# HeyWeCome/WhisprRec

Measured on AMD Instinct MI355X. Metric: BPR training triplets/sec, higher is better.
Workload: dtype f32; 1 GPU; BPRMF emb_size=64, synthetic 1000000 users x 1000000 items (uniform ids), batch 65536, SGD l2=0, plan build in timed region; batch=65536, emb_size=64, optimizer=SGD, plan_chunk_batches=64, tables=single GPU, step_stream=whisprrec_amd.hip_ops.PipelinedSgd, plan=group plan (no per-batch sort: flags + lists of the shared rows, wr_group.hip), chained_step_launch=True, plan_build=on a side stream, beside the steps of the chunk before

## Files before the change

### include/whisprrec_hip.h

```cpp
#ifndef WHISPRREC_HIP_H
#define WHISPRREC_HIP_H

#include <stdint.h>

#ifdef __cplusplus
extern "C" {
#endif

#define WR_ABI_VERSION 1

#define WR_OK 0
#define WR_E_NULL (-1)
#define WR_E_SHAPE (-2)
#define WR_E_WORKSPACE (-3)
#define WR_E_ALIGN (-4)
#define WR_E_RANGE (-5)

int32_t wr_abi_version(void);
const char *wr_last_error(void);
int32_t wr_device_info(int32_t *n_cu, int32_t *wave_size, char *arch, int32_t arch_len);

int64_t wr_bpr_fwd_workspace_bytes(int64_t B);
int32_t wr_bpr_fwd(const float *user_tab, int64_t n_users, const float *item_tab, int64_t n_items, int32_t D,
                   const int64_t *u, const int64_t *p, const int64_t *n, int64_t B, float *pos_score, float *neg_score,
// ... 5 lines not shown
                                int32_t *tn, int32_t *torig, int32_t *oc_item, int32_t *oc_src, int32_t *err_flag,
                                void *workspace, int64_t workspace_bytes, void *stream);
int32_t wr_bprmf_plan_build_i32(const int32_t *u, const int32_t *p, const int32_t *n, int64_t n_triplets,
                                int64_t batch_size, int64_t n_users, int64_t n_items, int32_t *tu, int32_t *tp,
                                int32_t *tn, int32_t *torig, int32_t *oc_item, int32_t *oc_src, int32_t *err_flag,
                                void *workspace, int64_t workspace_bytes, void *stream);

int64_t wr_bprmf_plan_small_max_batch(void);
int32_t wr_bprmf_plan_build_small_i64(const int64_t *u, const int64_t *p, const int64_t *n, int64_t n_triplets,
                                      int64_t batch_size, int64_t n_users, int64_t n_items, int32_t *tu, int32_t *tp,
                                      int32_t *tn, int32_t *torig, int32_t *oc_item, int32_t *oc_src, int32_t *err_flag,
                                      void *stream);
int32_t wr_bprmf_plan_build_small_i32(const int32_t *u, const int32_t *p, const int32_t *n, int64_t n_triplets,
                                      int64_t batch_size, int64_t n_users, int64_t n_items, int32_t *tu, int32_t *tp,
                                      int32_t *tn, int32_t *torig, int32_t *oc_item, int32_t *oc_src, int32_t *err_flag,
                                      void *stream);

int64_t wr_bprmf_plan_fast_workspace_bytes(int64_t n_triplets, int64_t batch_size, int64_t n_users, int64_t n_items);
int32_t wr_bprmf_plan_build_fast_i64(const int64_t *u, const int64_t *p, const int64_t *n, int64_t n_triplets,
                                     int64_t batch_size, int64_t n_users, int64_t n_items, int32_t *tu, int32_t *tp,
                                     int32_t *tn, int32_t *torig, int32_t *oc_item, int32_t *oc_src, int32_t *flags,
                                     void *workspace, int64_t workspace_bytes, void *stream);
int32_t wr_bprmf_plan_build_fast_i32(const int32_t *u, const int32_t *p, const int32_t *n, int64_t n_triplets,
                                     int64_t batch_size, int64_t n_users, int64_t n_items, int32_t *tu, int32_t *tp,
                                     int32_t *tn, int32_t *torig, int32_t *oc_item, int32_t *oc_src, int32_t *flags,
                                     void *workspace, int64_t workspace_bytes, void *stream);

int32_t wr_bprmf_plan_fast_marks_supported(int64_t n_triplets, int64_t batch_size, int64_t n_users, int64_t n_items);
int32_t wr_bprmf_plan_build_fast_marks_i64(const int64_t *u, const int64_t *p, const int64_t *n, int64_t n_triplets,
                                           int64_t batch_size, int64_t n_users, int64_t n_items, int32_t *tu, int32_t *tp,
                                           int32_t *tn, int32_t *torig, int32_t *oc_item, int32_t *oc_src, int32_t *flags,
                                           void *workspace, int64_t workspace_bytes, int32_t *bitmap, void *stream);
int32_t wr_bprmf_plan_build_fast_marks_i32(const int32_t *u, const int32_t *p, const int32_t *n, int64_t n_triplets,
                                           int64_t batch_size, int64_t n_users, int64_t n_items, int32_t *tu, int32_t *tp,
                                           int32_t *tn, int32_t *torig, int32_t *oc_item, int32_t *oc_src, int32_t *flags,
                                           void *workspace, int64_t workspace_bytes, int32_t *bitmap, void *stream);

typedef struct wr_bucket_side {
    int32_t n_buckets;
    const int32_t *row_bucket;
    const int32_t *bucket_start;
    const int32_t *bucket_rows;
    const int32_t *bucket_sub;
} wr_bucket_side;

int64_t wr_bprmf_plan_fast_mapped_workspace_bytes(int64_t n_triplets, int64_t batch_size, int64_t n_users, int64_t n_items,
                                                  int32_t n_buckets_users, int32_t n_buckets_items);
int32_t wr_bprmf_plan_build_fast_mapped_i64(const int64_t *u, const int64_t *p, const int64_t *n, int64_t n_triplets,
                                            int64_t batch_size, int64_t n_users, int64_t n_items,
                                            const wr_bucket_side *map_users, const wr_bucket_side *map_items, int32_t *tu,
                                            int32_t *tp, int32_t *tn, int32_t *torig, int32_t *oc_item, int32_t *oc_src,
                                            int32_t *flags, void *workspace, int64_t workspace_bytes, void *stream);
int32_t wr_bprmf_plan_build_fast_mapped_i32(const int32_t *u, const int32_t *p, const int32_t *n, int64_t n_triplets,
                                            int64_t batch_size, int64_t n_users, int64_t n_items,
                                            const wr_bucket_side *map_users, const wr_bucket_side *map_items, int32_t *tu,
                                            int32_t *tp, int32_t *tn, int32_t *torig, int32_t *oc_item, int32_t *oc_src,
                                            int32_t *flags, void *workspace, int64_t workspace_bytes, void *stream);

int32_t wr_sample_negatives_i64(const int64_t *users, int64_t n, int64_t n_users, int64_t n_items, const int64_t *clicked_ptr,
                                const int32_t *clicked_idx, uint64_t seed, uint64_t epoch, int64_t *neg_items,
                                int32_t *err_flag, void *stream);
int32_t wr_sample_negatives_i32(const int32_t *users, int64_t n, int64_t n_users, int64_t n_items, const int64_t *clicked_ptr,
                                const int32_t *clicked_idx, uint64_t seed, uint64_t epoch, int32_t *neg_items,
                                int32_t *err_flag, void *stream);

int32_t wr_epoch_prepare_range_i64(const int64_t *users, const int64_t *items, int64_t n, int64_t n_users, int64_t n_items,
                                   const int64_t *clicked_ptr, const int32_t *clicked_idx, uint64_t seed, uint64_t epoch,
                                   int64_t first, int64_t count, int64_t *out_users, int64_t *out_pos, int64_t *out_neg,
                                   int64_t *order_out, int32_t *err_flag, void *stream);
int32_t wr_epoch_prepare_range_i32(const int32_t *users, const int32_t *items, int64_t n, int64_t n_users, int64_t n_items,
                                   const int64_t *clicked_ptr, const int32_t *clicked_idx, uint64_t seed, uint64_t epoch,
                                   int64_t first, int64_t count, int32_t *out_users, int32_t *out_pos, int32_t *out_neg,
                                   int64_t *order_out, int32_t *err_flag, void *stream);

int64_t wr_pairset_capacity(int64_t n_pairs);
int32_t wr_pairset_build(const int64_t *clicked_ptr, const int32_t *clicked_idx, int64_t n_users, uint64_t *table,
                         int64_t capacity, int32_t *err_flag, void *stream);
int32_t wr_sample_negatives_set_i64(const int64_t *users, int64_t n, int64_t n_users, int64_t n_items, const uint64_t *pair_table,
                                    int64_t pair_capacity, uint64_t seed, uint64_t epoch, int64_t *neg_items,
                                    int32_t *err_flag, void *stream);
int32_t wr_sample_negatives_set_i32(const int32_t *users, int64_t n, int64_t n_users, int64_t n_items, const uint64_t *pair_table,
                                    int64_t pair_capacity, uint64_t seed, uint64_t epoch, int32_t *neg_items,
                                    int32_t *err_flag, void *stream);
int32_t wr_epoch_prepare_range_set_i64(const int64_t *users, const int64_t *items, int64_t n, int64_t n_users, int64_t n_items,
                                       const uint64_t *pair_table, int64_t pair_capacity, uint64_t seed, uint64_t epoch,
                                       int64_t first, int64_t count, int64_t *out_users, int64_t *out_pos, int64_t *out_neg,
                                       int64_t *order_out, int32_t *err_flag, void *stream);
int32_t wr_epoch_prepare_range_set_i32(const int32_t *users, const int32_t *items, int64_t n, int64_t n_users, int64_t n_items,
                                       const uint64_t *pair_table, int64_t pair_capacity, uint64_t seed, uint64_t epoch,
                                       int64_t first, int64_t count, int32_t *out_users, int32_t *out_pos, int32_t *out_neg,
                                       int64_t *order_out, int32_t *err_flag, void *stream);

int32_t wr_epoch_prepare_range_packed_i64(const uint64_t *packed_rows, int64_t n, int64_t n_users, int64_t n_items,
                                          const uint64_t *pair_table, int64_t pair_capacity, uint64_t seed, uint64_t epoch,
                                          int64_t first, int64_t count, int64_t *out_users, int64_t *out_pos, int64_t *out_neg,
                                          int64_t *order_out, int32_t *err_flag, void *stream);
int32_t wr_epoch_prepare_range_packed_i32(const uint64_t *packed_rows, int64_t n, int64_t n_users, int64_t n_items,
                                          const uint64_t *pair_table, int64_t pair_capacity, uint64_t seed, uint64_t epoch,
                                          int64_t first, int64_t count, int32_t *out_users, int32_t *out_pos, int32_t *out_neg,
                                          int64_t *order_out, int32_t *err_flag, void *stream);

int32_t wr_epoch_shuffle_i64(const int64_t *col0, const int64_t *col1, const int64_t *col2, int64_t n, uint64_t seed,
                             uint64_t epoch, int64_t *out0, int64_t *out1, int64_t *out2, int64_t *order_out, void *stream);
int32_t wr_epoch_shuffle_i32(const int32_t *col0, const int32_t *col1, const int32_t *col2, int64_t n, uint64_t seed,
                             uint64_t epoch, int32_t *out0, int32_t *out1, int32_t *out2, int64_t *order_out, void *stream);

typedef struct wr_hot_runs {
    const int32_t *piece_q, *piece_len, *run_q, *run_first, *run_np;
    const int32_t *u_piece_q, *u_piece_len, *u_run_q, *u_run_first, *u_run_np;
    const int32_t *counts_host;
    int64_t cap_pieces, cap_runs, cap_u_pieces, cap_u_runs;
} wr_hot_runs;
void wr_bprmf_hot_caps(int64_t batch_size, int32_t kind, int64_t *cap_pieces, int64_t *cap_runs);
int32_t wr_bprmf_plan_hot_runs(const int32_t *keys, int32_t kind, int64_t n_triplets, int64_t batch_size, int32_t *piece_q,
                               int32_t *piece_len, int32_t *run_q, int32_t *run_first, int32_t *run_np, int32_t *counts,
                               void *stream);

int64_t wr_bprmf_step_workspace_bytes(int64_t B, int32_t D);
int32_t wr_bprmf_step_sgd(float *user_tab, int64_t n_users, float *item_tab, int64_t n_items, int32_t D,
                          const int32_t *tu, const int32_t *tp, const int32_t *tn, const int32_t *oc_item,
                          const int32_t *oc_src, int64_t B, float lr, float l2, int32_t *stamp_u, int32_t *stamp_i,
                          int32_t step_id, float *loss_out, const wr_hot_runs *hot, void *workspace,
                          int64_t workspace_bytes, void *stream);

int32_t wr_bprmf_run_sgd(float *user_tab, int64_t n_users, float *item_tab, int64_t n_items, int32_t D,
                         const int32_t *tu, const int32_t *tp, const int32_t *tn, const int32_t *oc_item,
                         const int32_t *oc_src, int64_t n_triplets, int64_t batch_size, int64_t first_batch,
                         int64_t n_batches, float lr, float *loss_out, void *const *phase_events, const wr_hot_runs *hot,
                         void *workspace, int64_t workspace_bytes, void *stream);

int32_t wr_bprmf_chain_supported(const float *user_tab, const float *item_tab, int32_t D);
int64_t wr_bprmf_chain_sync_words(int64_t n_batches);
int32_t wr_bprmf_run_sgd_chain(float *user_tab, int64_t n_users, float *item_tab, int64_t n_items, int32_t D,
                               const int32_t *tu, const int32_t *tp, const int32_t *tn, const int32_t *oc_item,
                               const int32_t *oc_src, int64_t n_triplets, int64_t batch_size, int64_t first_batch,
                               int64_t n_batches, float lr, float *loss_out, const int32_t *tdef, const int32_t *def_q,
                               const int32_t *def_count_host, int64_t def_cap, int64_t def_limit, void *const *phase_events,
                               void *workspace, int64_t workspace_bytes, int32_t *sync, int64_t sync_words, void *stream);

int64_t wr_group_plan_words(int64_t n_triplets, int64_t batch_size, int64_t n_users, int64_t n_items);
int32_t wr_group_plan_layout(int64_t n_triplets, int64_t batch_size, int64_t n_users, int64_t n_items, int64_t *out);
int32_t wr_narrow_ids_i64(const int64_t *u, const int64_t *p, const int64_t *n, int32_t *u32, int32_t *p32, int32_t *n32,
                          int64_t count, void *stream);
int32_t wr_group_plan_build(const int32_t *u, const int32_t *p, const int32_t *n, int64_t n_triplets, int64_t batch_size,
                            int64_t n_users, int64_t n_items, int32_t *plan, int64_t plan_words, void *stream);
int64_t wr_bprmf_group_workspace_bytes(int64_t batch_size, int32_t D);
int64_t wr_bprmf_group_sync_words(int64_t n_batches);
int32_t wr_bprmf_group_supported(const float *user_tab, const float *item_tab, int32_t D);
int32_t wr_bprmf_run_sgd_group(float *user_tab, int64_t n_users, float *item_tab, int64_t n_items, int32_t D,
                               const int32_t *u, const int32_t *p, const int32_t *n, int64_t n_triplets, int64_t batch_size,
                               const int32_t *plan, int64_t plan_words, int64_t first_batch, int64_t n_batches, float lr,
                               float *loss_out, void *const *events, void *workspace, int64_t workspace_bytes, int32_t *sync,
                               int64_t sync_words, void *stream);

int32_t wr_bprmf_plan_overlap_marks(const int32_t *tu, const int32_t *tp, const int32_t *tn, int64_t n_triplets,
                                    int64_t batch_size, int64_t n_items, const int32_t *prev_bitmap, int32_t *bitmap,
                                    int32_t *tdef, int32_t *def_q, int64_t def_cap, int32_t *def_count, void *stream);

int32_t wr_bprmf_plan_overlap_deferred(const int32_t *tu, const int32_t *tp, const int32_t *tn, int64_t n_triplets,
                                       int64_t batch_size, int64_t n_items, const int32_t *prev_bitmap, const int32_t *bitmap,
                                       int32_t *tdef, int32_t *def_q, int64_t def_cap, int32_t *def_count, void *stream);

int32_t wr_bprmf_grads(const float *user_tab, int64_t n_users, const float *item_tab, int64_t n_items, int32_t D,
                       const int32_t *tu, const int32_t *tp, const int32_t *tn, const int32_t *oc_item,
                       const int32_t *oc_src, int64_t B, float *grad_u, float *grad_i, int32_t *stamp_u,
                       int32_t *stamp_i, int32_t step_id, float *loss_out, const wr_hot_runs *hot, void *workspace,
                       int64_t workspace_bytes, void *stream);

int32_t wr_sgd_decay_untouched(float *tab, int64_t n_rows, int32_t D, const int32_t *stamp, int32_t step_id, float lr,
                               float l2, void *stream);
int32_t wr_sgd_dense(float *tab, int64_t n_rows, int32_t D, const float *grad, const int32_t *stamp, int32_t step_id,
                     float lr, float l2, void *stream);
int32_t wr_adam_dense(float *tab, float *exp_avg, float *exp_avg_sq, int64_t n_rows, int32_t D, const float *grad,
                      const int32_t *stamp, int32_t step_id, int64_t adam_step, float lr, float l2, float beta1,
                      float beta2, float eps, void *stream);

int32_t wr_adam_dense_dev(float *tab, float *exp_avg, float *exp_avg_sq, int64_t n_rows, int32_t D, const float *grad,
                          const float *consts, int64_t n_consts, const int32_t *step_dev, float l2, float beta1, float beta2,
                          float eps, void *stream);

int32_t wr_adam_dense_dev_pair(float *tab_a, float *exp_avg_a, float *exp_avg_sq_a, int64_t n_rows_a, const float *grad_a,
                               float *tab_b, float *exp_avg_b, float *exp_avg_sq_b, int64_t n_rows_b, const float *grad_b,
                               int32_t D, const float *consts, int64_t n_consts, const int32_t *step_dev, float l2,
                               float beta1, float beta2, float eps, void *stream);
int32_t wr_counter_add(int32_t *counter, int32_t delta, void *stream);

int32_t wr_adam_consts(int64_t first_step, int64_t n_steps, float lr, float beta1, float beta2, float *consts_host);
int32_t wr_adam_rows_lazy(float *tab, float *exp_avg, float *exp_avg_sq, int32_t *last_step, int64_t n_rows, int32_t D,
                          const int32_t *keys, int64_t n_keys, const float *grad, int64_t adam_step, const float *consts,
                          int64_t n_consts, float l2, float beta1, float beta2, float eps, void *stream);
int32_t wr_adam_catchup_all(float *tab, float *exp_avg, float *exp_avg_sq, int32_t *last_step, int64_t n_rows, int32_t D,
                            int64_t adam_step, const float *consts, int64_t n_consts, float l2, float beta1, float beta2,
                            float eps, void *stream);
int32_t wr_sgd_rows_lazy(float *tab, int32_t *last_step, int64_t n_rows, int32_t D, const int32_t *keys, int64_t n_keys,
                         int64_t step, float lr, float l2, void *stream);
int32_t wr_sgd_catchup_all(float *tab, int32_t *last_step, int64_t n_rows, int32_t D, int64_t step, float lr, float l2,
                           void *stream);

int32_t wr_bprmf_step_adam(float *user_tab, int64_t n_users, float *item_tab, int64_t n_items, int32_t D, float *m_u,
                           float *v_u, float *m_i, float *v_i, int32_t *last_u, int32_t *last_i, const int32_t *tu,
                           const int32_t *tp, const int32_t *tn, const int32_t *oc_item, const int32_t *oc_src, int64_t B,
                           int64_t adam_step, float lr, float l2, float beta1, float beta2, float eps, float *loss_out,
                           const wr_hot_runs *hot, void *workspace, int64_t workspace_bytes, void *stream);
int32_t wr_bprmf_run_stateful(int32_t kind, float *user_tab, int64_t n_users, float *item_tab, int64_t n_items, int32_t D,
                              float *s1_u, float *s2_u, float *s1_i, float *s2_i, int32_t *last_u, int32_t *last_i,
                              const int32_t *tu, const int32_t *tp, const int32_t *tn, const int32_t *oc_item,
                              const int32_t *oc_src, int64_t n_triplets, int64_t batch_size, int64_t first_batch,
                              int64_t n_batches, int64_t step0, float lr, float rho, float eps, float *loss_out,
                              const wr_hot_runs *hot, void *workspace, int64_t workspace_bytes, void *stream);
int32_t wr_bprmf_step_adam_folded(float *user_tab, int64_t n_users, float *item_tab, int64_t n_items, int32_t D, float *m_u,
                                  float *v_u, float *m_i, float *v_i, int32_t *last_u, int32_t *last_i, const int32_t *tu,
                                  const int32_t *tp, const int32_t *tn, const int32_t *oc_item, const int32_t *oc_src,
                                  int64_t B, int64_t adam_step, float lr, const float *consts, int64_t n_consts, float l2,
                                  float beta1, float beta2, float eps, float *loss_out, void *workspace,
                                  int64_t workspace_bytes, void *stream);
int32_t wr_bprmf_run_adam_folded(float *user_tab, int64_t n_users, float *item_tab, int64_t n_items, int32_t D, float *m_u,
                                 float *v_u, float *m_i, float *v_i, int32_t *last_u, int32_t *last_i, const int32_t *tu,
                                 const int32_t *tp, const int32_t *tn, const int32_t *oc_item, const int32_t *oc_src,
                                 int64_t n_triplets, int64_t batch_size, int64_t first_batch, int64_t n_batches,
                                 int64_t adam_step0, float lr, const float *consts, int64_t n_consts, float l2, float beta1,
                                 float beta2, float eps, float *loss_out, const wr_hot_runs *hot, void *workspace,
                                 int64_t workspace_bytes, void *stream);
int32_t wr_bprmf_run_adam_folded_chain(float *user_tab, int64_t n_users, float *item_tab, int64_t n_items, int32_t D,
                                       float *m_u, float *v_u, float *m_i, float *v_i, int32_t *last_u, int32_t *last_i,
                                       const int32_t *tu, const int32_t *tp, const int32_t *tn, const int32_t *oc_item,
                                       const int32_t *oc_src, int64_t n_triplets, int64_t batch_size, int64_t first_batch,
                                       int64_t n_batches, int64_t adam_step0, float lr, const float *consts, int64_t n_consts,
                                       float l2, float beta1, float beta2, float eps, float *loss_out, const int32_t *tdef,
                                       const int32_t *def_q, const int32_t *def_count_host, int64_t def_cap, int64_t def_limit,
                                       void *workspace, int64_t workspace_bytes, int32_t *sync, int64_t sync_words,
                                       void *stream);
int32_t wr_bprmf_run_adam_lazy_bounded(float *user_tab, int64_t n_users, float *item_tab, int64_t n_items, int32_t D,
                                       float *m_u, float *v_u, float *m_i, float *v_i, int32_t *last_u, int32_t *last_i,
                                       const int32_t *tu, const int32_t *tp, const int32_t *tn, const int32_t *oc_item,
                                       const int32_t *oc_src, int64_t n_triplets, int64_t batch_size, int64_t first_batch,
                                       int64_t n_batches, int64_t adam_step0, float lr, const float *consts, int64_t n_consts,
                                       float l2, float beta1, float beta2, float eps, float *loss_out, const wr_hot_runs *hot,
                                       int64_t max_lag, int64_t *sweep_pos, void *workspace, int64_t workspace_bytes,
                                       void *stream);
int32_t wr_bprmf_run_sgd_lazy_bounded(float *user_tab, int64_t n_users, float *item_tab, int64_t n_items, int32_t D,
                                      int32_t *last_u, int32_t *last_i, int32_t *stamp_u, int32_t *stamp_i, int32_t step_id0,
                                      const int32_t *tu, const int32_t *tp, const int32_t *tn, const int32_t *oc_item,
                                      const int32_t *oc_src, int64_t n_triplets, int64_t batch_size, int64_t first_batch,
                                      int64_t n_batches, int64_t step0, float lr, float l2, float *loss_out,
                                      const wr_hot_runs *hot, int64_t max_lag, int64_t *sweep_pos, void *workspace,
                                      int64_t workspace_bytes, void *stream);
int32_t wr_bprmf_run_stateful_bounded(int32_t kind, float *user_tab, int64_t n_users, float *item_tab, int64_t n_items,
                                      int32_t D, float *s1_u, float *s2_u, float *s1_i, float *s2_i, int32_t *last_u,
                                      int32_t *last_i, const int32_t *tu, const int32_t *tp, const int32_t *tn,
                                      const int32_t *oc_item, const int32_t *oc_src, int64_t n_triplets, int64_t batch_size,
                                      int64_t first_batch, int64_t n_batches, int64_t step0, float lr, float rho, float eps,
                                      float *loss_out, const wr_hot_runs *hot, int64_t max_lag, int64_t *sweep_pos,
                                      void *workspace, int64_t workspace_bytes, void *stream);
int32_t wr_adadelta_decay_all(float *square_avg, float *acc_delta, int32_t *last_step, int64_t n_rows, int32_t D, int64_t step,
                              float rho, void *stream);
int32_t wr_bprmf_run_adam_lazy(float *user_tab, int64_t n_users, float *item_tab, int64_t n_items, int32_t D, float *m_u,
                               float *v_u, float *m_i, float *v_i, int32_t *last_u, int32_t *last_i, const int32_t *tu,
                               const int32_t *tp, const int32_t *tn, const int32_t *oc_item, const int32_t *oc_src,
                               int64_t n_triplets, int64_t batch_size, int64_t first_batch, int64_t n_batches,
                               int64_t adam_step0, float lr, const float *consts, int64_t n_consts, float l2, float beta1,
                               float beta2, float eps, float *loss_out, const wr_hot_runs *hot, void *workspace,
                               int64_t workspace_bytes, void *stream);
int32_t wr_bprmf_run_sgd_lazy(float *user_tab, int64_t n_users, float *item_tab, int64_t n_items, int32_t D, int32_t *last_u,
                              int32_t *last_i, int32_t *stamp_u, int32_t *stamp_i, int32_t step_id0, const int32_t *tu,
                              const int32_t *tp, const int32_t *tn, const int32_t *oc_item, const int32_t *oc_src,
                              int64_t n_triplets, int64_t batch_size, int64_t first_batch, int64_t n_batches, int64_t step0,
                              float lr, float l2, float *loss_out, const wr_hot_runs *hot, void *workspace,
                              int64_t workspace_bytes, void *stream);

int32_t wr_gather_rows(const float *tab, int64_t n_rows, int32_t D, const int64_t *idx, int64_t n, float *out,
                       void *stream);
int64_t wr_scatter_add_workspace_bytes(int64_t n, int64_t n_rows);
int32_t wr_scatter_add_rows(float *grad, int64_t n_rows, int32_t D, const int64_t *idx, const float *src, int64_t n,
                            int64_t padding_idx, float alpha, void *workspace, int64_t workspace_bytes, void *stream);

int64_t wr_scatter_plan_words(int64_t n_segments, int64_t seg_stride, int64_t n_rows);
int32_t wr_scatter_plan_build(const int64_t *idx, int64_t n_segments, int64_t seg_stride, const int32_t *seg_len, int64_t n_rows,
                              int64_t padding_idx, int32_t *plan, int64_t plan_words, void *stream);
int32_t wr_scatter_add_planned(float *table, int64_t n_rows, int32_t D, const int64_t *idx, int64_t n_segments,
                               int64_t seg_stride, int64_t segment, int64_t n, int64_t padding_idx, const float *src,
                               float alpha, const int32_t *plan, int64_t plan_words, void *stream);

int32_t wr_apply_rows_sorted(float *tab, int64_t n_rows, int32_t D, const int32_t *sorted_rows, const int32_t *perm,
                             const float *src, int64_t n, float alpha, void *stream);

int32_t wr_bprmf_shard_step(float *user_shard, int64_t n_user_rows, float *item_rows, int64_t n_rows, int64_t n_local_items,
                            int32_t D, const int32_t *tu, const int32_t *tp, const int32_t *tn, const int32_t *oc_item,
                            const int32_t *oc_src, int64_t B, int64_t global_batch, float lr, float *grad_slots,
                            float *loss_partial, const wr_hot_runs *hot, void *workspace, int64_t workspace_bytes,
                            void *stream);

int32_t wr_shard_route(const int32_t *u, const int32_t *p, const int32_t *n, int64_t n_triplets, int64_t batch_size, int32_t world,
                       int32_t rank, int64_t n_users, int64_t n_items, int64_t rows_per_owner, int64_t n_local_items,
                       int64_t list_cap, int32_t *vu, int32_t *vp, int32_t *vn, int32_t *send_rows, int32_t *send_cnt,
                       int32_t *err, void *stream);
int32_t wr_shard_pack(const int32_t *recv_rows, const int32_t *recv_cnt, int64_t n_batches, int32_t world, int64_t list_cap,
                      int64_t n_local_items, int64_t *serve_rows, int64_t serve_stride, int32_t *serve_off, int32_t *err,
                      void *stream);
int32_t wr_bprmf_shard_step_group(float *user_shard, int64_t n_user_rows, float *item_ext, int64_t n_ext_rows,
                                  int64_t n_local_items, int32_t D, const int32_t *vu, const int32_t *vp, const int32_t *vn,
                                  int64_t n_triplets, int64_t batch_size, const int32_t *plan, int64_t plan_words, int64_t batch,
                                  int64_t global_batch, float lr, float *grad_slots, float *loss_partial, void *workspace,
                                  int64_t workspace_bytes, int32_t *sync, int64_t sync_words, void *stream);

int32_t wr_spmm_csr(int64_t n_rows, const int64_t *row_ptr, const int32_t *col, const float *val, const float *X,
                    int32_t D, float *Y, float *acc, void *stream);
// ... 145 lines not shown
```

### whisprrec_amd/abi.py

```python
import ctypes
import os

_HERE = os.path.dirname(os.path.abspath(__file__))
LIB_PATH = os.path.join(_HERE, "libwhisprrec_hip.so")

c_i32, c_i64, c_f32, c_vp = ctypes.c_int32, ctypes.c_int64, ctypes.c_float, ctypes.c_void_p

SIGNATURES = {
    "wr_abi_version": (c_i32, []),
    "wr_last_error": (ctypes.c_char_p, []),
    "wr_device_info": (c_i32, [c_vp, c_vp, c_vp, c_i32]),
    "wr_bpr_fwd_workspace_bytes": (c_i64, [c_i64]),
    "wr_bpr_fwd": (c_i32, [c_vp, c_i64, c_vp, c_i64, c_i32, c_vp, c_vp, c_vp, c_i64, c_vp, c_vp, c_vp, c_vp, c_vp, c_i64,
                           c_vp]),
    "wr_bprmf_plan_workspace_bytes": (c_i64, [c_i64, c_i64, c_i64, c_i64]),
    "wr_bprmf_plan_build_i64": (c_i32, [c_vp, c_vp, c_vp, c_i64, c_i64, c_i64, c_i64, c_vp, c_vp, c_vp, c_vp, c_vp, c_vp,
                                        c_vp, c_vp, c_i64, c_vp]),
    "wr_bprmf_plan_build_i32": (c_i32, [c_vp, c_vp, c_vp, c_i64, c_i64, c_i64, c_i64, c_vp, c_vp, c_vp, c_vp, c_vp, c_vp,
                                        c_vp, c_vp, c_i64, c_vp]),
    "wr_bprmf_plan_small_max_batch": (c_i64, []),
    "wr_bprmf_plan_build_small_i64": (c_i32, [c_vp, c_vp, c_vp, c_i64, c_i64, c_i64, c_i64, c_vp, c_vp, c_vp, c_vp, c_vp, c_vp,
                                              c_vp, c_vp]),
    "wr_bprmf_plan_build_small_i32": (c_i32, [c_vp, c_vp, c_vp, c_i64, c_i64, c_i64, c_i64, c_vp, c_vp, c_vp, c_vp, c_vp, c_vp,
                                              c_vp, c_vp]),
    "wr_bprmf_plan_fast_workspace_bytes": (c_i64, [c_i64, c_i64, c_i64, c_i64]),
    "wr_bprmf_plan_fast_mapped_workspace_bytes": (c_i64, [c_i64, c_i64, c_i64, c_i64, c_i32, c_i32]),
    "wr_bprmf_plan_build_fast_mapped_i64": (c_i32, [c_vp, c_vp, c_vp, c_i64, c_i64, c_i64, c_i64, c_vp, c_vp, c_vp, c_vp, c_vp,
                                                    c_vp, c_vp, c_vp, c_vp, c_vp, c_i64, c_vp]),
    "wr_bprmf_plan_build_fast_mapped_i32": (c_i32, [c_vp, c_vp, c_vp, c_i64, c_i64, c_i64, c_i64, c_vp, c_vp, c_vp, c_vp, c_vp,
                                                    c_vp, c_vp, c_vp, c_vp, c_vp, c_i64, c_vp]),
    "wr_bprmf_plan_build_fast_i64": (c_i32, [c_vp, c_vp, c_vp, c_i64, c_i64, c_i64, c_i64, c_vp, c_vp, c_vp, c_vp, c_vp,
                                             c_vp, c_vp, c_vp, c_i64, c_vp]),
    "wr_bprmf_plan_build_fast_i32": (c_i32, [c_vp, c_vp, c_vp, c_i64, c_i64, c_i64, c_i64, c_vp, c_vp, c_vp, c_vp, c_vp,
                                             c_vp, c_vp, c_vp, c_i64, c_vp]),
    "wr_sample_negatives_i64": (c_i32, [c_vp, c_i64, c_i64, c_i64, c_vp, c_vp, ctypes.c_uint64, ctypes.c_uint64, c_vp, c_vp,
                                        c_vp]),
    "wr_sample_negatives_i32": (c_i32, [c_vp, c_i64, c_i64, c_i64, c_vp, c_vp, ctypes.c_uint64, ctypes.c_uint64, c_vp, c_vp,
                                        c_vp]),
    "wr_epoch_prepare_range_i64": (c_i32, [c_vp, c_vp, c_i64, c_i64, c_i64, c_vp, c_vp, ctypes.c_uint64, ctypes.c_uint64, c_i64, c_i64,
                                           c_vp, c_vp, c_vp, c_vp, c_vp, c_vp]),
    "wr_epoch_prepare_range_i32": (c_i32, [c_vp, c_vp, c_i64, c_i64, c_i64, c_vp, c_vp, ctypes.c_uint64, ctypes.c_uint64, c_i64, c_i64,
                                           c_vp, c_vp, c_vp, c_vp, c_vp, c_vp]),
    "wr_pairset_capacity": (c_i64, [c_i64]),
    "wr_pairset_build": (c_i32, [c_vp, c_vp, c_i64, c_vp, c_i64, c_vp, c_vp]),
    "wr_sample_negatives_set_i64": (c_i32, [c_vp, c_i64, c_i64, c_i64, c_vp, c_i64, ctypes.c_uint64, ctypes.c_uint64, c_vp, c_vp,
                                            c_vp]),
    "wr_sample_negatives_set_i32": (c_i32, [c_vp, c_i64, c_i64, c_i64, c_vp, c_i64, ctypes.c_uint64, ctypes.c_uint64, c_vp, c_vp,
                                            c_vp]),
    "wr_epoch_prepare_range_set_i64": (c_i32, [c_vp, c_vp, c_i64, c_i64, c_i64, c_vp, c_i64, ctypes.c_uint64, ctypes.c_uint64, c_i64,
                                               c_i64, c_vp, c_vp, c_vp, c_vp, c_vp, c_vp]),
    "wr_epoch_prepare_range_set_i32": (c_i32, [c_vp, c_vp, c_i64, c_i64, c_i64, c_vp, c_i64, ctypes.c_uint64, ctypes.c_uint64, c_i64,
                                               c_i64, c_vp, c_vp, c_vp, c_vp, c_vp, c_vp]),
    "wr_epoch_prepare_range_packed_i64": (c_i32, [c_vp, c_i64, c_i64, c_i64, c_vp, c_i64, ctypes.c_uint64, ctypes.c_uint64, c_i64,
                                                  c_i64, c_vp, c_vp, c_vp, c_vp, c_vp, c_vp]),
    "wr_epoch_prepare_range_packed_i32": (c_i32, [c_vp, c_i64, c_i64, c_i64, c_vp, c_i64, ctypes.c_uint64, ctypes.c_uint64, c_i64,
                                                  c_i64, c_vp, c_vp, c_vp, c_vp, c_vp, c_vp]),
    "wr_epoch_shuffle_i64": (c_i32, [c_vp, c_vp, c_vp, c_i64, ctypes.c_uint64, ctypes.c_uint64, c_vp, c_vp, c_vp, c_vp, c_vp]),
    "wr_epoch_shuffle_i32": (c_i32, [c_vp, c_vp, c_vp, c_i64, ctypes.c_uint64, ctypes.c_uint64, c_vp, c_vp, c_vp, c_vp, c_vp]),
    "wr_bprmf_step_workspace_bytes": (c_i64, [c_i64, c_i32]),
    "wr_bprmf_hot_caps": (None, [c_i64, c_i32, c_vp, c_vp]),
    "wr_bprmf_plan_hot_runs": (c_i32, [c_vp, c_i32, c_i64, c_i64, c_vp, c_vp, c_vp, c_vp, c_vp, c_vp, c_vp]),
    "wr_bprmf_step_sgd": (c_i32, [c_vp, c_i64, c_vp, c_i64, c_i32, c_vp, c_vp, c_vp, c_vp, c_vp, c_i64, c_f32, c_f32,
                                  c_vp, c_vp, c_i32, c_vp, c_vp, c_vp, c_i64, c_vp]),
    "wr_bprmf_run_sgd": (c_i32, [c_vp, c_i64, c_vp, c_i64, c_i32, c_vp, c_vp, c_vp, c_vp, c_vp, c_i64, c_i64, c_i64,
                                 c_i64, c_f32, c_vp, c_vp, c_vp, c_vp, c_i64, c_vp]),
    "wr_bprmf_chain_supported": (c_i32, [c_vp, c_vp, c_i32]),
    "wr_bprmf_chain_sync_words": (c_i64, [c_i64]),
    "wr_bprmf_run_sgd_chain": (c_i32, [c_vp, c_i64, c_vp, c_i64, c_i32, c_vp, c_vp, c_vp, c_vp, c_vp, c_i64, c_i64, c_i64,
                                       c_i64, c_f32, c_vp, c_vp, c_vp, c_vp, c_i64, c_i64, c_vp, c_vp, c_i64, c_vp, c_i64,
                                       c_vp]),
    "wr_lightgcn_step_workspace_bytes": (c_i64, [c_i64, c_i64, c_i32, c_i64, c_i64]),
    "wr_lightgcn_step": (c_i32, [c_vp, c_vp, c_i64, c_i64, c_i32, c_i64, c_vp, c_vp, c_vp, c_vp, c_i32, c_i32, c_vp, c_vp, c_vp,
                                 c_i64, c_f32, c_i32, c_vp, c_vp, c_vp, c_vp, c_i64, c_vp]),
    "wr_shard_route": (c_i32, [c_vp, c_vp, c_vp, c_i64, c_i64, c_i32, c_i32, c_i64, c_i64, c_i64, c_i64, c_i64, c_vp, c_vp, c_vp,
                               c_vp, c_vp, c_vp, c_vp]),
    "wr_shard_pack": (c_i32, [c_vp, c_vp, c_i64, c_i32, c_i64, c_i64, c_vp, c_i64, c_vp, c_vp, c_vp]),
    "wr_bprmf_shard_step_group": (c_i32, [c_vp, c_i64, c_vp, c_i64, c_i64, c_i32, c_vp, c_vp, c_vp, c_i64, c_i64, c_vp, c_i64,
                                          c_i64, c_i64, c_f32, c_vp, c_vp, c_vp, c_i64, c_vp, c_i64, c_vp]),
    "wr_group_plan_words": (c_i64, [c_i64, c_i64, c_i64, c_i64]),
    "wr_group_plan_layout": (c_i32, [c_i64, c_i64, c_i64, c_i64, c_vp]),
    "wr_narrow_ids_i64": (c_i32, [c_vp, c_vp, c_vp, c_vp, c_vp, c_vp, c_i64, c_vp]),
    "wr_group_plan_build": (c_i32, [c_vp, c_vp, c_vp, c_i64, c_i64, c_i64, c_i64, c_vp, c_i64, c_vp]),
    "wr_bprmf_group_workspace_bytes": (c_i64, [c_i64, c_i32]),
    "wr_bprmf_group_sync_words": (c_i64, [c_i64]),
    "wr_bprmf_group_supported": (c_i32, [c_vp, c_vp, c_i32]),
    "wr_bprmf_run_sgd_group": (c_i32, [c_vp, c_i64, c_vp, c_i64, c_i32, c_vp, c_vp, c_vp, c_i64, c_i64, c_vp, c_i64, c_i64,
                                       c_i64, c_f32, c_vp, c_vp, c_vp, c_i64, c_vp, c_i64, c_vp]),
    "wr_bprmf_plan_overlap_deferred": (c_i32, [c_vp, c_vp, c_vp, c_i64, c_i64, c_i64, c_vp, c_vp, c_vp, c_vp, c_i64, c_vp,
                                               c_vp]),
    "wr_bprmf_plan_fast_marks_supported": (c_i32, [c_i64, c_i64, c_i64, c_i64]),
    "wr_bprmf_plan_build_fast_marks_i64": (c_i32, [c_vp, c_vp, c_vp, c_i64, c_i64, c_i64, c_i64, c_vp, c_vp, c_vp, c_vp, c_vp,
                                                   c_vp, c_vp, c_vp, c_i64, c_vp, c_vp]),
    "wr_bprmf_plan_build_fast_marks_i32": (c_i32, [c_vp, c_vp, c_vp, c_i64, c_i64, c_i64, c_i64, c_vp, c_vp, c_vp, c_vp, c_vp,
                                                   c_vp, c_vp, c_vp, c_i64, c_vp, c_vp]),
    "wr_bprmf_plan_overlap_marks": (c_i32, [c_vp, c_vp, c_vp, c_i64, c_i64, c_i64, c_vp, c_vp, c_vp, c_vp, c_i64, c_vp,
                                            c_vp]),
    "wr_bprmf_grads": (c_i32, [c_vp, c_i64, c_vp, c_i64, c_i32, c_vp, c_vp, c_vp, c_vp, c_vp, c_i64, c_vp, c_vp, c_vp,
                               c_vp, c_i32, c_vp, c_vp, c_vp, c_i64, c_vp]),
    "wr_sgd_decay_untouched": (c_i32, [c_vp, c_i64, c_i32, c_vp, c_i32, c_f32, c_f32, c_vp]),
    "wr_sgd_dense": (c_i32, [c_vp, c_i64, c_i32, c_vp, c_vp, c_i32, c_f32, c_f32, c_vp]),
    "wr_adam_dense": (c_i32, [c_vp, c_vp, c_vp, c_i64, c_i32, c_vp, c_vp, c_i32, c_i64, c_f32, c_f32, c_f32, c_f32,
                              c_f32, c_vp]),
    "wr_adam_dense_dev": (c_i32, [c_vp, c_vp, c_vp, c_i64, c_i32, c_vp, c_vp, c_i64, c_vp, c_f32, c_f32, c_f32, c_f32, c_vp]),
    "wr_adam_dense_dev_pair": (c_i32, [c_vp, c_vp, c_vp, c_i64, c_vp, c_vp, c_vp, c_vp, c_i64, c_vp, c_i32, c_vp, c_i64, c_vp,
                                       c_f32, c_f32, c_f32, c_f32, c_vp]),
    "wr_counter_add": (c_i32, [c_vp, c_i32, c_vp]),
    "wr_adam_consts": (c_i32, [c_i64, c_i64, c_f32, c_f32, c_f32, c_vp]),
    "wr_adam_rows_lazy": (c_i32, [c_vp, c_vp, c_vp, c_vp, c_i64, c_i32, c_vp, c_i64, c_vp, c_i64, c_vp, c_i64, c_f32, c_f32,
                                  c_f32, c_f32, c_vp]),
    "wr_adam_catchup_all": (c_i32, [c_vp, c_vp, c_vp, c_vp, c_i64, c_i32, c_i64, c_vp, c_i64, c_f32, c_f32, c_f32, c_f32,
                                    c_vp]),
    "wr_sgd_rows_lazy": (c_i32, [c_vp, c_vp, c_i64, c_i32, c_vp, c_i64, c_i64, c_f32, c_f32, c_vp]),
    "wr_sgd_catchup_all": (c_i32, [c_vp, c_vp, c_i64, c_i32, c_i64, c_f32, c_f32, c_vp]),
    "wr_bprmf_step_adam": (c_i32, [c_vp, c_i64, c_vp, c_i64, c_i32, c_vp, c_vp, c_vp, c_vp, c_vp, c_vp, c_vp, c_vp, c_vp, c_vp, c_vp,
                                   c_i64, c_i64, c_f32, c_f32, c_f32, c_f32, c_f32, c_vp, c_vp, c_vp, c_i64, c_vp]),
    "wr_bprmf_run_stateful": (c_i32, [c_i32, c_vp, c_i64, c_vp, c_i64, c_i32, c_vp, c_vp, c_vp, c_vp, c_vp, c_vp, c_vp, c_vp, c_vp,
                                      c_vp, c_vp, c_i64, c_i64, c_i64, c_i64, c_i64, c_f32, c_f32, c_f32, c_vp, c_vp, c_vp, c_i64,
                                      c_vp]),
    "wr_bprmf_step_adam_folded": (c_i32, [c_vp, c_i64, c_vp, c_i64, c_i32, c_vp, c_vp, c_vp, c_vp, c_vp, c_vp, c_vp, c_vp, c_vp, c_vp,
                                          c_vp, c_i64, c_i64, c_f32, c_vp, c_i64, c_f32, c_f32, c_f32, c_f32, c_vp, c_vp, c_i64,
                                          c_vp]),
    "wr_bprmf_run_adam_folded": (c_i32, [c_vp, c_i64, c_vp, c_i64, c_i32, c_vp, c_vp, c_vp, c_vp, c_vp, c_vp, c_vp, c_vp, c_vp, c_vp,
                                         c_vp, c_i64, c_i64, c_i64, c_i64, c_i64, c_f32, c_vp, c_i64, c_f32, c_f32, c_f32, c_f32,
                                         c_vp, c_vp, c_vp, c_i64, c_vp]),
    "wr_bprmf_run_adam_folded_chain": (c_i32, [c_vp, c_i64, c_vp, c_i64, c_i32, c_vp, c_vp, c_vp, c_vp, c_vp, c_vp, c_vp, c_vp, c_vp,
                                               c_vp, c_vp, c_i64, c_i64, c_i64, c_i64, c_i64, c_f32, c_vp, c_i64, c_f32, c_f32,
                                               c_f32, c_f32, c_vp, c_vp, c_vp, c_vp, c_i64, c_i64, c_vp, c_i64, c_vp, c_i64,
                                               c_vp]),
    "wr_bprmf_run_sgd_lazy_bounded": (c_i32, [c_vp, c_i64, c_vp, c_i64, c_i32, c_vp, c_vp, c_vp, c_vp, c_i32, c_vp, c_vp, c_vp,
                                              c_vp, c_vp, c_i64, c_i64, c_i64, c_i64, c_i64, c_f32, c_f32, c_vp, c_vp, c_i64,
                                              c_vp, c_vp, c_i64, c_vp]),
    "wr_bprmf_run_stateful_bounded": (c_i32, [c_i32, c_vp, c_i64, c_vp, c_i64, c_i32, c_vp, c_vp, c_vp, c_vp, c_vp, c_vp, c_vp,
                                              c_vp, c_vp, c_vp, c_vp, c_i64, c_i64, c_i64, c_i64, c_i64, c_f32, c_f32, c_f32,
                                              c_vp, c_vp, c_i64, c_vp, c_vp, c_i64, c_vp]),
    "wr_adadelta_decay_all": (c_i32, [c_vp, c_vp, c_vp, c_i64, c_i32, c_i64, c_f32, c_vp]),
    "wr_bprmf_run_adam_lazy_bounded": (c_i32, [c_vp, c_i64, c_vp, c_i64, c_i32, c_vp, c_vp, c_vp, c_vp, c_vp, c_vp, c_vp, c_vp,
                                               c_vp, c_vp, c_vp, c_i64, c_i64, c_i64, c_i64, c_i64, c_f32, c_vp, c_i64, c_f32,
                                               c_f32, c_f32, c_f32, c_vp, c_vp, c_i64, c_vp, c_vp, c_i64, c_vp]),
    "wr_bprmf_run_adam_lazy": (c_i32, [c_vp, c_i64, c_vp, c_i64, c_i32, c_vp, c_vp, c_vp, c_vp, c_vp, c_vp, c_vp, c_vp, c_vp, c_vp,
                                       c_vp, c_i64, c_i64, c_i64, c_i64, c_i64, c_f32, c_vp, c_i64, c_f32, c_f32, c_f32, c_f32,
                                       c_vp, c_vp, c_vp, c_i64, c_vp]),
    "wr_bprmf_run_sgd_lazy": (c_i32, [c_vp, c_i64, c_vp, c_i64, c_i32, c_vp, c_vp, c_vp, c_vp, c_i32, c_vp, c_vp, c_vp, c_vp, c_vp,
                                      c_i64, c_i64, c_i64, c_i64, c_i64, c_f32, c_f32, c_vp, c_vp, c_vp, c_i64, c_vp]),
    "wr_gather_rows": (c_i32, [c_vp, c_i64, c_i32, c_vp, c_i64, c_vp, c_vp]),
    "wr_scatter_add_workspace_bytes": (c_i64, [c_i64, c_i64]),
    "wr_scatter_add_rows": (c_i32, [c_vp, c_i64, c_i32, c_vp, c_vp, c_i64, c_i64, c_f32, c_vp, c_i64, c_vp]),
    "wr_scatter_plan_words": (c_i64, [c_i64, c_i64, c_i64]),
    "wr_scatter_plan_build": (c_i32, [c_vp, c_i64, c_i64, c_vp, c_i64, c_i64, c_vp, c_i64, c_vp]),
    "wr_scatter_add_planned": (c_i32, [c_vp, c_i64, c_i32, c_vp, c_i64, c_i64, c_i64, c_i64, c_i64, c_vp, c_f32, c_vp, c_i64,
                                       c_vp]),
    "wr_apply_rows_sorted": (c_i32, [c_vp, c_i64, c_i32, c_vp, c_vp, c_vp, c_i64, c_f32, c_vp]),
    "wr_bprmf_shard_step": (c_i32, [c_vp, c_i64, c_vp, c_i64, c_i64, c_i32, c_vp, c_vp, c_vp, c_vp, c_vp, c_i64, c_i64, c_f32,
                                    c_vp, c_vp, c_vp, c_vp, c_i64, c_vp]),
    "wr_spmm_csr": (c_i32, [c_i64, c_vp, c_vp, c_vp, c_vp, c_i32, c_vp, c_vp, c_vp]),
    "wr_spmm_csr_chunked": (c_i32, [c_i64, c_i64, c_vp, c_vp, c_vp, c_vp, c_vp, c_i32, c_vp, c_vp, c_vp, c_vp]),
    "wr_spmm_dense_partials_bytes": (c_i64, [c_i64, c_i64, c_i64, c_i32]),
    "wr_spmm_dense_tiles": (c_i32, [c_vp, c_vp, c_vp, c_i64, c_i32, c_vp, c_vp, c_vp]),
    "wr_spmm_csr_chunked_levels": (c_i32, [c_i64, c_i64, c_vp, c_vp, c_vp, c_vp, c_vp, c_i32, c_vp, c_vp, c_vp, c_vp, c_i32,
                                           c_i32, c_f32, c_vp]),
    "wr_spmm_fused_supported": (c_i32, [c_i32, c_vp]),
    "wr_spmm_csr_chunked_fused": (c_i32, [c_i64, c_i64, c_vp, c_vp, c_vp, c_vp, c_vp, c_vp, c_i32, c_vp, c_vp, c_vp, c_vp, c_i32,
                                          c_f32, c_vp, c_vp]),
    "wr_spmm_csr_chunked_modes": (c_i32, [c_i64, c_i64, c_vp, c_vp, c_vp, c_vp, c_vp, c_i32, c_vp, c_vp, c_vp, c_vp, c_vp]),
    "wr_axpy": (c_i32, [c_vp, c_vp, c_i64, c_f32, c_i32, c_vp]),
    "wr_rank_eval": (c_i32, [c_vp, c_i64, c_vp, c_i64, c_i32, c_vp, c_vp, c_i64, c_vp, c_vp, c_vp, c_vp, c_vp]),
    "wr_rank_eval_rows": (c_i32, [c_vp, c_i64, c_vp, c_i64, c_i32, c_vp, c_vp, c_i64, c_vp, c_i64, c_vp, c_vp, c_vp, c_vp, c_vp]),
    "wr_topk_supported": (c_i32, [c_i32, c_i32]),
    "wr_topk_workspace_bytes": (c_i64, [c_i64, c_i64, c_i32, c_i32]),
    "wr_topk_recommend": (c_i32, [c_vp, c_i64, c_vp, c_i64, c_i32, c_vp, c_i64, c_vp, c_vp, c_i32, c_vp, c_vp, c_vp, c_i64,
                                  c_vp]),
    "wr_topk_recommend_rows": (c_i32, [c_vp, c_i64, c_vp, c_i64, c_i32, c_vp, c_i64, c_vp, c_i64, c_vp, c_vp, c_i32, c_vp, c_vp, c_vp,
                                       c_i64, c_vp]),
    "wr_infonce_supported": (c_i32, [c_i32]),
    "wr_infonce_workspace_bytes": (c_i64, [c_i64, c_i64, c_i32]),
    "wr_infonce_loss_grad": (c_i32, [c_vp, c_vp, c_i64, c_i32, c_vp, c_i64, c_f32, c_f32, c_vp, c_i32, c_vp, c_vp, c_vp, c_vp,
                                     c_i64, c_vp]),
    "wr_sasblock_supported": (c_i32, [c_i32, c_i32, c_i32, c_i32]),
    "wr_sasblock_workspace_bytes": (c_i64, [c_i64, c_i32, c_i32, c_i32, c_i32]),
    "wr_sasblock_fwd": (c_i32, [c_vp, c_i64, c_i32, c_i32, c_i32, c_i32, c_vp, c_f32, ctypes.c_uint64, c_i32, c_vp, c_vp, c_vp, c_i64,
                                c_vp]),
    "wr_sasblock_bwd": (c_i32, [c_vp, c_vp, c_i64, c_i32, c_i32, c_i32, c_i32, c_vp, c_f32, ctypes.c_uint64, c_i32, c_vp, c_vp, c_vp,
                                c_vp, c_i64, c_vp]),
    "wr_sasblock_fwd_keys": (c_i32, [c_vp, c_i64, c_i32, c_i32, c_i32, c_i32, c_vp, c_f32, ctypes.c_uint64, c_i32, c_vp, c_vp, c_vp,
                                     c_i64, c_vp, c_vp, c_vp]),
    "wr_sasblock_bwd_keys": (c_i32, [c_vp, c_vp, c_i64, c_i32, c_i32, c_i32, c_i32, c_vp, c_f32, ctypes.c_uint64, c_i32, c_vp, c_vp,
                                     c_vp, c_vp, c_i64, c_vp, c_vp, c_vp]),
    "wr_supcon_supported": (c_i32, [c_i32]),
    "wr_supcon_workspace_bytes": (c_i64, [c_i64, c_i32]),
    "wr_supcon_loss_grad": (c_i32, [c_vp, c_i64, c_i32, c_vp, c_f32, c_vp, c_i32, c_f32, c_vp, c_vp, c_vp, c_i64, c_vp]),
    "wr_buir_supported": (c_i32, [c_i32]),
    "wr_buir_workspace_bytes": (c_i64, [c_i64, c_i32]),
    "wr_buir_loss_grad": (c_i32, [c_vp, c_vp, c_vp, c_vp, c_i64, c_i64, c_i32, c_vp, c_vp, c_vp, c_vp, c_i64, c_vp, c_vp, c_vp, c_vp,
                                  c_vp, c_vp, c_vp, c_i64, c_vp]),
    "wr_ema_update": (c_i32, [c_vp, c_vp, c_i64, c_f32, c_f32, c_vp]),
    "wr_interest_pool_supported": (c_i32, [c_i32, c_i32, c_i32, c_i32]),
    "wr_interest_pool_workspace_bytes": (c_i64, [c_i64, c_i32, c_i32, c_i32, c_i32]),
    "wr_interest_pool_fwd": (c_i32, [c_vp, c_i64, c_vp, c_i64, c_i32, c_vp, c_i64, c_i32, c_vp, c_vp, c_vp, c_vp, c_i32, c_i32, c_vp,
                                     c_vp, c_vp]),
    "wr_interest_pool_bwd": (c_i32, [c_vp, c_i64, c_vp, c_i64, c_i32, c_vp, c_i64, c_i32, c_vp, c_vp, c_vp, c_vp, c_i32, c_i32, c_vp,
                                     c_vp, c_vp, c_vp, c_vp, c_vp, c_vp, c_vp, c_vp, c_i64, c_vp]),
    "wr_rank_eval_multi_supported": (c_i32, [c_i32, c_i32]),
    "wr_rank_eval_multi": (c_i32, [c_vp, c_i64, c_vp, c_i64, c_i32, c_i32, c_vp, c_i64, c_vp, c_i64, c_vp, c_vp, c_vp, c_vp, c_vp]),
    "wr_sgl_views_workspace_bytes": (c_i64, [c_i64, c_i64]),
    "wr_sgl_view_count": (c_i32, [c_i32, c_vp, c_vp, c_vp, c_i64, c_i64, c_vp, c_i64, c_i64, ctypes.c_uint64, ctypes.c_uint64,
                                  ctypes.c_uint64, c_vp, c_vp, c_vp, c_vp, c_i64, c_vp]),
    "wr_sgl_view_rows": (c_i32, [c_vp, c_i64, c_i64, c_vp, c_vp, c_vp, c_vp, c_vp]),
    "wr_sgl_view_fill": (c_i32, [c_vp, c_vp, c_vp, c_i64, c_i64, c_vp, c_i64, c_vp, c_vp, c_vp, c_vp, c_i64, c_vp, c_vp, c_i64,
                                 c_vp, c_vp, c_i64, c_vp, c_vp, c_i64, c_vp]),
    "wr_spmm_chunks_count": (c_i32, [c_vp, c_i64, c_i32, c_vp, c_vp, c_vp]),
    "wr_spmm_chunks_fill": (c_i32, [c_vp, c_i64, c_i32, c_vp, c_i64, c_vp, c_vp, c_vp]),
    "wr_lightgcn_loss_workspace_bytes": (c_i64, [c_i64]),
    "wr_lightgcn_loss": (c_i32, [c_vp, c_vp, c_vp, c_vp, c_i64, c_i64, c_i32, c_vp, c_vp, c_vp, c_i64, c_f32, c_vp, c_vp, c_vp,
                                 c_i64, c_vp]),
    "wr_embloss_grad": (c_i32, [c_vp, c_vp, c_i32, c_vp, c_vp, c_vp, c_i64, c_vp, c_f32, c_vp, c_vp, c_vp]),
    "wr_embloss_sumsq": (c_i32, [c_vp, c_vp, c_i32, c_vp, c_vp, c_vp, c_i64, c_vp, c_vp, c_i64, c_vp]),
}



class HotRuns(ctypes.Structure):
    _fields_ = [("piece_q", c_vp), ("piece_len", c_vp), ("run_q", c_vp), ("run_first", c_vp), ("run_np", c_vp),
                ("u_piece_q", c_vp), ("u_piece_len", c_vp), ("u_run_q", c_vp), ("u_run_first", c_vp), ("u_run_np", c_vp),
                ("counts_host", c_vp), ("cap_pieces", c_i64), ("cap_runs", c_i64), ("cap_u_pieces", c_i64),
                ("cap_u_runs", c_i64)]


class DenseGroup(ctypes.Structure):
    _fields_ = [("A_T", c_vp), ("cols", c_vp), ("rows", c_vp), ("partials", c_vp), ("K_pad", c_i64), ("k_per_split", c_i64),
                ("n_tiles", c_i64)]


class BucketSide(ctypes.Structure):
    _fields_ = [("n_buckets", c_i32), ("row_bucket", c_vp), ("bucket_start", c_vp), ("bucket_rows", c_vp), ("bucket_sub", c_vp)]


_lib = None


class WhisprRecHipError(RuntimeError):
    pass


def lib():
    global _lib
    if _lib is None:
        if not os.path.exists(LIB_PATH):
            raise WhisprRecHipError(
                "libwhisprrec_hip.so is missing at %s — build it with `python -c 'import __graft_entry__ as g; g.build()'` "
                "or `make -C whisprrec_amd/csrc`.  There is no CPU fallback." % LIB_PATH)
        import torch
        handle = ctypes.CDLL(LIB_PATH)
        for name, (res, args) in SIGNATURES.items():
            fn = getattr(handle, name)
            fn.restype = res
            fn.argtypes = args
        if handle.wr_abi_version() != 1:
            raise WhisprRecHipError("ABI version mismatch: library %d, binding 1" % handle.wr_abi_version())
        _lib = handle
    return _lib


def last_error():
    return lib().wr_last_error().decode("utf-8", "replace")


def check(rc, what):
    if rc != 0:
        raise WhisprRecHipError("%s failed (rc=%d): %s" % (what, rc, last_error()))


def check_size(nbytes, what):
    if nbytes < 0:
        raise WhisprRecHipError("%s failed (rc=%d): %s" % (what, nbytes, last_error()))
    return int(nbytes)
```

### whisprrec_amd/csrc/wr_group.hip

```cpp
#include "wr_common.h"
#include <hip/hip_ext.h>

#include <algorithm>

namespace wr {

constexpr int kGpThreads = 1024;
constexpr unsigned kGpRangeBits = 18;
constexpr int kGpWords = 1 << (kGpRangeBits - 5);
constexpr int kGpCap = 8192;
constexpr int kGpBins = 4096;
constexpr int kGpMaxBin = 256;
constexpr int kGpMaxRanges = 8;
constexpr int64_t kGpMaxBatch = 1 << 17;
constexpr int kGpLongRun = 64;
constexpr int kGpMetaWords = 16;
#ifndef WR_GP_DBG
#define WR_GP_DBG 0
#endif

struct GroupLayout {
    int64_t nb, B, fw;
    int R_u, R_i, cap_u, cap_i;
    unsigned mask_u, mask_i, hbits_u, hbits_i;
    int64_t flags, ucnt, icnt, ul_row, ul_src, il_row, il_src, total;
    int64_t zero_words;
};

static inline int ranges_for(int64_t n_rows, unsigned *mask, unsigned *hbits, int *cap) {
    unsigned bits = kGpRangeBits;
    while (bits < kGpRangeBits + 3 && (int64_t(1) << bits) < n_rows) ++bits;
    *mask = (1u << bits) - 1u;
    *hbits = bits;
    const int R = 1 << (bits - kGpRangeBits);
    *cap = kGpCap;
    return R;
}

static bool group_layout(int64_t n, int64_t B, int64_t n_users, int64_t n_items, GroupLayout &L) {
    if (n <= 0 || n >= (int64_t(1) << 31) || B <= 0 || B > kGpMaxBatch) return false;
    if (n_users <= 0 || n_users >= (int64_t(1) << 31) || n_items <= 0 || n_items >= (int64_t(1) << 31)) return false;
    L.nb = (n + B - 1) / B;
    L.B = B;
    L.fw = (B + 31) / 32;
    L.R_u = ranges_for(n_users, &L.mask_u, &L.hbits_u, &L.cap_u);
    L.R_i = ranges_for(n_items, &L.mask_i, &L.hbits_i, &L.cap_i);
    L.flags = kGpMetaWords;
    L.ucnt = L.flags + L.nb * L.fw * 4;
    L.icnt = L.ucnt + align_up(L.nb * L.R_u, 4);
    L.zero_words = L.icnt + align_up(L.nb * L.R_i, 4);
    L.ul_row = L.zero_words;
    L.ul_src = L.ul_row + L.nb * L.R_u * (int64_t)L.cap_u;
    L.il_row = L.ul_src + L.nb * L.R_u * (int64_t)L.cap_u;
    L.il_src = L.il_row + L.nb * L.R_i * (int64_t)L.cap_i;
    L.total = L.il_src + L.nb * L.R_i * (int64_t)L.cap_i;
    return true;
}

struct GpDev {
    int *meta;
    unsigned *flags;
    int *ucnt, *icnt;
    int *ul_row, *ul_src, *il_row, *il_src;
    int R_u, R_i, cap_u, cap_i;
    unsigned mask_u, mask_i, hbits_u, hbits_i;
    int fw;
};

static inline GpDev group_dev(int32_t *plan, const GroupLayout &L) {
    return GpDev{plan, reinterpret_cast<unsigned *>(plan + L.flags), plan + L.ucnt, plan + L.icnt, plan + L.ul_row,
                 plan + L.ul_src, plan + L.il_row, plan + L.il_src, L.R_u, L.R_i, L.cap_u, L.cap_i, L.mask_u, L.mask_i,
                 L.hbits_u, L.hbits_i, (int)L.fw};
}

template <typename F>
__device__ __forceinline__ void gp_scan(const int *__restrict__ a, int cnt, F f) {
    if ((reinterpret_cast<uintptr_t>(a) & 15u) == 0) {
        const int n4 = cnt >> 2;
        const int4 *a4 = reinterpret_cast<const int4 *>(a);
        int i = threadIdx.x;
        for (; i + 3 * kGpThreads < n4; i += 4 * kGpThreads) {
            int4 v[4];
#pragma unroll
            for (int q = 0; q < 4; ++q) v[q] = a4[i + q * kGpThreads];
#pragma unroll
            for (int q = 0; q < 4; ++q) {
                const int at = 4 * (i + q * kGpThreads);
                f(v[q].x, at);
                f(v[q].y, at + 1);
                f(v[q].z, at + 2);
                f(v[q].w, at + 3);
            }
        }
        for (; i < n4; i += kGpThreads) {
            const int4 v = a4[i];
            f(v.x, 4 * i);
            f(v.y, 4 * i + 1);
            f(v.z, 4 * i + 2);
            f(v.w, 4 * i + 3);
        }
        for (int j = (n4 << 2) + threadIdx.x; j < cnt; j += kGpThreads) f(a[j], j);
    } else {
        for (int j = threadIdx.x; j < cnt; j += kGpThreads) f(a[j], j);
    }
}

__global__ __launch_bounds__(kGpThreads) void group_plan_kernel(const int *__restrict__ u, const int *__restrict__ p,
                                                                 const int *__restrict__ n, int64_t n_total, int B, int nb,
                                                                 int n_users, int n_items, GpDev L) {
    extern __shared__ __attribute__((aligned(16))) unsigned gp_lds[];
    unsigned *seen = gp_lds;
    unsigned long long *keys = reinterpret_cast<unsigned long long *>(gp_lds);
    unsigned *multi = gp_lds + 2 * kGpCap;
    unsigned *f0 = multi + kGpWords, *f1 = f0 + L.fw, *f2 = f1 + L.fw;
    int &n_list = *reinterpret_cast<int *>(f2 + L.fw);
    const int per = L.R_u + L.R_i;
    const unsigned lb = xcd_contiguous_id(blockIdx.x, gridDim.x);
    const int b = (int)(lb / (unsigned)per), rr = (int)(lb % (unsigned)per);
    const bool item = rr >= L.R_u;
    const unsigned r = (unsigned)(item ? rr - L.R_u : rr);
    const int64_t base = (int64_t)b * B;
    const int Bb = (int)((base + B <= n_total) ? B : (n_total - base));
    const unsigned n_rows = (unsigned)(item ? n_items : n_users);
    const unsigned mask = item ? L.mask_i : L.mask_u;
    const unsigned rb = (item ? L.hbits_i : L.hbits_u) - kGpRangeBits, rsel = (1u << rb) - 1u;
    for (int i = threadIdx.x; i < kGpWords; i += kGpThreads) {
        seen[i] = 0u;
        multi[i] = 0u;
    }
    for (int i = threadIdx.x; i < 3 * L.fw; i += kGpThreads) f0[i] = 0u;
    if (threadIdx.x == 0) n_list = 0;
    __syncthreads();
    auto mark = [&](int row, int) {
        if ((unsigned)row >= n_rows) {
            L.meta[0] = 1;
            return;
        }
        const unsigned h = (unsigned)row & mask;
        if ((h & rsel) != r) return;
        const unsigned bit = h >> rb, m = 1u << (bit & 31u);
        const unsigned old = atomicOr(&seen[bit >> 5], m);
        if (old & m) atomicOr(&multi[bit >> 5], m);
    };
    if (!(WR_GP_DBG & 8)) {
        if (item) {
            gp_scan(p + base, Bb, mark);
            gp_scan(n + base, Bb, mark);
        } else {
            gp_scan(u + base, Bb, mark);
        }
    }
    __syncthreads();
    auto several = [&](int row) -> bool {
        const unsigned h = (unsigned)row & mask;
        if ((h & rsel) != r) return false;
        const unsigned bit = h >> rb;
        return (multi[bit >> 5] >> (bit & 31u)) & 1u;
    };
    auto append = [&](int row, unsigned src) {
        const int pos = atomicAdd(&n_list, 1);
        if (pos < kGpCap) keys[pos] = ((unsigned long long)(unsigned)row << 32) | src;
    };
    if (!(WR_GP_DBG & 2)) {
        const bool next = b + 1 < nb && !(WR_GP_DBG & 16);
        const int64_t nbase = base + B;
        const int Bn = next ? (int)((nbase + B <= n_total) ? B : (n_total - nbase)) : 0;
        auto defer = [&](int row, int t) {
            if (several(row)) atomicOr(&f2[t >> 5], 1u << (t & 31));
        };
        if (item) {
            gp_scan(p + base, Bb, [&](int row, int t) {
                if (several(row)) {
                    atomicOr(&f0[t >> 5], 1u << (t & 31));
                    append(row, (unsigned)t << 1);
                }
            });
            gp_scan(n + base, Bb, [&](int row, int t) {
                if (several(row)) {
                    atomicOr(&f1[t >> 5], 1u << (t & 31));
                    append(row, ((unsigned)t << 1) | 1u);
                }
            });
            gp_scan(p + nbase, Bn, defer);
            gp_scan(n + nbase, Bn, defer);
        } else {
            gp_scan(u + base, Bb, [&](int row, int t) {
                if (several(row)) {
                    atomicOr(&f0[t >> 5], 1u << (t & 31));
                    append(row, (unsigned)t << 1);
                }
            });
            gp_scan(u + nbase, Bn, defer);
        }
    }
    __syncthreads();
    if (!(WR_GP_DBG & 4)) {
        unsigned *fb = L.flags + (int64_t)b * L.fw * 4;
        for (int w = threadIdx.x; w < L.fw; w += kGpThreads) {
            if (f0[w]) __hip_atomic_fetch_or(fb + 4 * w + (item ? 1 : 0), f0[w], __ATOMIC_RELAXED, __HIP_MEMORY_SCOPE_AGENT);
            if (item && f1[w]) __hip_atomic_fetch_or(fb + 4 * w + 2, f1[w], __ATOMIC_RELAXED, __HIP_MEMORY_SCOPE_AGENT);
            if (f2[w])
                __hip_atomic_fetch_or(fb + 4 * (L.fw + w) + 3, f2[w], __ATOMIC_RELAXED, __HIP_MEMORY_SCOPE_AGENT);
        }
    }
    const int cap = item ? L.cap_i : L.cap_u, R = item ? L.R_i : L.R_u;
    int m = n_list;
    if (m > cap) {
        if (threadIdx.x == 0) L.meta[1] = 1;
        m = cap;
    }
    int *cnt = reinterpret_cast<int *>(multi);
    unsigned short *out16 = reinterpret_cast<unsigned short *>(multi + kGpBins);
    int *wave_tot = reinterpret_cast<int *>(f0);
    auto bin_of = [&](unsigned long long k) -> int { return (int)(((((unsigned)(k >> 32)) & mask) >> rb) & (kGpBins - 1)); };
    int *lrow = (item ? L.il_row : L.ul_row) + ((int64_t)b * R + r) * cap, *lsrc = (item ? L.il_src : L.ul_src) + ((int64_t)b * R + r) * cap;
    __syncthreads();
    for (int i = threadIdx.x; i < kGpBins; i += kGpThreads) cnt[i] = 0;
    __syncthreads();
    if (!(WR_GP_DBG & 1)) {
        for (int j = threadIdx.x; j < m; j += kGpThreads) atomicAdd(&cnt[bin_of(keys[j])], 1);
        __syncthreads();
        constexpr int kOwn = kGpBins / kGpThreads;
        const int c0 = (int)threadIdx.x * kOwn;
        int local = 0;
#pragma unroll
        for (int j = 0; j < kOwn; ++j) local += cnt[c0 + j];
        int incl = local;
#pragma unroll
        for (int d = 1; d < 64; d <<= 1) {
            const int v = __shfl_up(incl, d, 64);
            if ((int)(threadIdx.x & 63) >= d) incl += v;
        }
        if ((threadIdx.x & 63) == 63) wave_tot[threadIdx.x >> 6] = incl;
        __syncthreads();
        int run = incl - local;
        for (int w = 0; w < (int)(threadIdx.x >> 6); ++w) run += wave_tot[w];
#pragma unroll
        for (int j = 0; j < kOwn; ++j) {
            const int c = cnt[c0 + j];
            cnt[c0 + j] = run;
            run += c;
        }
        __syncthreads();
        for (int j = threadIdx.x; j < m; j += kGpThreads) out16[atomicAdd(&cnt[bin_of(keys[j])], 1)] = (unsigned short)j;
        __syncthreads();
        for (int j = threadIdx.x; j < m; j += kGpThreads) {
            const unsigned long long k = keys[j];
            const int bin = bin_of(k);
            const int lo = bin ? cnt[bin - 1] : 0, hi = cnt[bin];
            if (hi - lo > kGpMaxBin) {
                L.meta[1] = 1;
                continue;
            }
            int pos = lo, same = 0;
            for (int jj = lo; jj < hi; ++jj) {
                const unsigned long long o = keys[out16[jj]];
                pos += o < k ? 1 : 0;
                same += (unsigned)(o >> 32) == (unsigned)(k >> 32) ? 1 : 0;
            }
            if (same > kGpLongRun) L.meta[2] = 1;
            lrow[pos] = (int)(k >> 32);
            lsrc[pos] = (int)(unsigned)k;
        }
    } else {
        for (int j = threadIdx.x; j < m; j += kGpThreads) {
            lrow[j] = (int)(keys[j] >> 32);
            lsrc[j] = (int)(unsigned)keys[j];
        }
    }
    if (threadIdx.x == 0) (item ? L.icnt : L.ucnt)[(int64_t)b * R + r] = m;
}

__global__ __launch_bounds__(kBlock) void narrow_ids_kernel(const int64_t *__restrict__ u, const int64_t *__restrict__ p,
                                                             const int64_t *__restrict__ n, int *__restrict__ u32,
                                                             int *__restrict__ p32, int *__restrict__ n32, int64_t cnt) {
    const int64_t i = (int64_t)blockIdx.x * kBlock + threadIdx.x;
    if (i >= cnt) return;
    const int64_t a = u[i], b = p[i], c = n[i];
    u32[i] = (a >= 0 && a < (int64_t(1) << 31)) ? (int)a : -1;
    p32[i] = (b >= 0 && b < (int64_t(1) << 31)) ? (int)b : -1;
    n32[i] = (c >= 0 && c < (int64_t(1) << 31)) ? (int)c : -1;
}

constexpr int kGsTile = 32;
constexpr int kGsAhead = 8;
constexpr int kGsShards = 64;
constexpr int kGsShardStride = 16;
constexpr int kGsStepWords = kGsShards * kGsShardStride;
constexpr int kGsDefChunk = 32;
constexpr int kGsLdsInts = 1024 + 8;
constexpr unsigned kGsSpinLimit = 1u << 22;

struct GsBatch {
    const int *u, *p, *n;
    const uint4 *flags;
    const int *ul_row, *ul_src, *ul_cnt, *il_row, *il_src, *il_cnt;
    int B, R_u, R_i, cap_u, cap_i;
};

struct GsArgs {
    float *U, *I;
    int D;
    float lr;
    GsBatch cur;
    float *Z, *ZU, *partials;
    float denom;
    GsBatch prev;
    const float *Zp, *ZUp, *partials_prev;
    int n_partials_prev;
    float denom_prev;
    float *loss_prev;
    int nA, nIT, nUT, nDS, tiles_at, side_at;
    int chained;
    unsigned *done, *timeout;
    float *Gs;
    int nL;
};

template <int NV>
__device__ __forceinline__ Row<NV> row_zero() {
    Row<NV> r;
#pragma unroll
    for (int k = 0; k < NV; ++k) r.v[k] = make_float4(0.f, 0.f, 0.f, 0.f);
    return r;
}

template <int T, int NV, bool FULL>
__device__ __forceinline__ void gs_single(const GsArgs &a, int t, int u, int p, int n, bool us, bool ps, bool ns, int lane,
                                          float &terms) {
    const Row<NV> ur = load_row<T, NV, FULL>(a.U, u, a.D, lane);
    const Row<NV> pr = load_row<T, NV, FULL>(a.I, p, a.D, lane);
    const Row<NV> nr = load_row<T, NV, FULL>(a.I, n, a.D, lane);
    const float sp = team_sum<T>(dot_partial<NV>(ur, pr));
    const float sn = team_sum<T>(dot_partial<NV>(ur, nr));
    float term, c;
    bpr_terms(sp, sn, a.denom, term, c);
    terms += term;
    Row<NV> g, z;
#pragma unroll
    for (int k = 0; k < NV; ++k) {
        g.v[k] = make_float4(c * (pr.v[k].x - nr.v[k].x), c * (pr.v[k].y - nr.v[k].y), c * (pr.v[k].z - nr.v[k].z),
                             c * (pr.v[k].w - nr.v[k].w));
        z.v[k] = make_float4(c * ur.v[k].x, c * ur.v[k].y, c * ur.v[k].z, c * ur.v[k].w);
    }
    const float lr = a.lr;
    if (!us) {
        Row<NV> w;
#pragma unroll
        for (int k = 0; k < NV; ++k)
            w.v[k] = make_float4(ur.v[k].x - lr * g.v[k].x, ur.v[k].y - lr * g.v[k].y, ur.v[k].z - lr * g.v[k].z,
                                 ur.v[k].w - lr * g.v[k].w);
        store_row<T, NV, FULL>(a.U, u, a.D, lane, w);
    } else {
        store_row<T, NV, FULL>(a.ZU, t, a.D, lane, g);
    }
    if (!ps) {
        if (a.Gs != nullptr && p >= a.nL) {
// ... 199 lines not shown
template <int T, int NV, bool FULL>
__global__ __launch_bounds__(kBlock, NV == 1 ? WR_GS_WAVES : 1) void bprmf_group_step(GsArgs a) {
    __shared__ float scratch[kBlock / 64];
    __shared__ __attribute__((aligned(16))) int lds[kGsLdsInts];
    constexpr int TEAMS = kBlock / T;
    const int lane = threadIdx.x % T;
    int b = (int)blockIdx.x;
    if (b >= a.tiles_at && b < a.tiles_at + a.nIT + a.nUT) {
        const int w = b - a.tiles_at;
        const bool wt = a.nA > 0;
        if (!(WR_GS_DBG & 1)) {
            if (w < a.nIT) {
                if (wt) gs_list_tiles<T, NV, FULL, true>(a.I, a.D, a.lr, a.prev.il_row, a.prev.il_src, a.prev.il_cnt, a.prev.R_i, a.prev.cap_i,
                                                         a.prev.B, a.Zp, w, a.nIT, lds, a.Gs, a.nL);
                else gs_list_tiles<T, NV, FULL, false>(a.I, a.D, a.lr, a.prev.il_row, a.prev.il_src, a.prev.il_cnt, a.prev.R_i, a.prev.cap_i,
                                                       a.prev.B, a.Zp, w, a.nIT, lds, a.Gs, a.nL);
            } else {
                if (wt) gs_list_tiles<T, NV, FULL, true>(a.U, a.D, a.lr, a.prev.ul_row, a.prev.ul_src, a.prev.ul_cnt, a.prev.R_u, a.prev.cap_u,
                                                         a.prev.B, a.ZUp, w - a.nIT, a.nUT, lds);
                else gs_list_tiles<T, NV, FULL, false>(a.U, a.D, a.lr, a.prev.ul_row, a.prev.ul_src, a.prev.ul_cnt, a.prev.R_u, a.prev.cap_u,
                                                       a.prev.B, a.ZUp, w - a.nIT, a.nUT, lds);
            }
        }
        if (wt) {
            asm volatile("s_waitcnt vmcnt(0)" ::: "memory");
            __syncthreads();
            if (threadIdx.x == 0)
                __hip_atomic_fetch_add(a.done + (w % kGsShards) * kGsShardStride, 1u, __ATOMIC_RELAXED, __HIP_MEMORY_SCOPE_AGENT);
        }
        if (w == 0 && a.loss_prev != nullptr) {
            const float s0 = strided_partial_sum(a.partials_prev, a.n_partials_prev);
            const float s = block_sum(s0, scratch);
            if (threadIdx.x == 0) a.loss_prev[0] = s / a.denom_prev;
        }
        return;
    }
    if (b >= a.tiles_at) b -= a.nIT + a.nUT;
    float terms = 0.f;
    int slot;
    if (b >= a.side_at && b < a.side_at + a.nDS) {
        const int w = b - a.side_at;
        int *dl = lds, &total_s = lds[kGsDefChunk * 32];
        const int fw = (a.cur.B + 31) / 32;
        const int per = (fw + a.nDS - 1) / a.nDS;
        const int w_end = min(fw, (w + 1) * per);
        bool waited = false;
        for (int c0 = w * per; c0 < w_end; c0 += kGsDefChunk) {
            const int wi = c0 + (int)threadIdx.x;
            unsigned m = 0u, us = 0u, ps = 0u, ns = 0u;
            if (threadIdx.x < kGsDefChunk && wi < w_end) {
                const uint4 f = a.cur.flags[wi];
                m = f.w;
                us = f.x;
                ps = f.y;
                ns = f.z;
            }
            int cnt = __popc(m), incl = cnt;
#pragma unroll
            for (int d = 1; d < 64; d <<= 1) {
                const int v = __shfl_up(incl, d, 64);
                if ((int)(threadIdx.x & 63) >= d) incl += v;
            }
            if (threadIdx.x == 63) total_s = incl;
            int at = incl - cnt;
            while (m) {
                const int bit = __ffs(m) - 1;
                m &= m - 1;
                dl[at++] = ((wi * 32 + bit) << 3) | (((us >> bit) & 1u) ? 4 : 0) | (((ps >> bit) & 1u) ? 1 : 0) |
                           (((ns >> bit) & 1u) ? 2 : 0);
            }
            __syncthreads();
            const int total = (WR_GS_DBG & 2) ? 0 : total_s;
            const int e0 = (int)threadIdx.x / T, e1 = e0 + TEAMS;
            int t0 = 0, u0 = 0, p0 = 0, n0 = 0, t1 = 0, u1 = 0, p1 = 0, n1 = 0;
            if (e0 < total) {
                t0 = min(dl[e0] >> 3, a.cur.B - 1);
                u0 = a.cur.u[t0];
                p0 = a.cur.p[t0];
                n0 = a.cur.n[t0];
            }
            if (e1 < total) {
                t1 = min(dl[e1] >> 3, a.cur.B - 1);
                u1 = a.cur.u[t1];
                p1 = a.cur.p[t1];
                n1 = a.cur.n[t1];
            }
            if (!waited) {
                if (!(WR_GS_DBG & 4)) gs_wait_tiles(a);
                waited = true;
            }
            if (e0 < total) gs_single<T, NV, FULL>(a, t0, u0, p0, n0, dl[e0] & 4, dl[e0] & 1, dl[e0] & 2, lane, terms);
            if (e1 < total) gs_single<T, NV, FULL>(a, t1, u1, p1, n1, dl[e1] & 4, dl[e1] & 1, dl[e1] & 2, lane, terms);
            for (int e = e1 + TEAMS; e < total; e += TEAMS) {
                const int t = min(dl[e] >> 3, a.cur.B - 1);
                gs_single<T, NV, FULL>(a, t, a.cur.u[t], a.cur.p[t], a.cur.n[t], dl[e] & 4, dl[e] & 1, dl[e] & 2, lane, terms);
            }
            __syncthreads();
        }
        slot = a.nA + w;
    } else {
        if (b >= a.side_at) b -= a.nDS;
        const int t = b * TEAMS + (int)threadIdx.x / T;
        const int tc = min(t, a.cur.B - 1);
        uint4 f = a.cur.flags[tc >> 5];
        int u = a.cur.u[tc], p = a.cur.p[tc], n = a.cur.n[tc];
#if WR_GS_DBG & 8
        f = make_uint4(0u, 0u, 0u, 0u);
#endif
        asm volatile("" : "+v"(u), "+v"(p), "+v"(n), "+v"(f.x), "+v"(f.y), "+v"(f.z), "+v"(f.w));
        const unsigned bit = 1u << (t & 31);
        if (t < a.cur.B && !(a.chained && (f.w & bit)))
            gs_single<T, NV, FULL>(a, t, u, p, n, f.x & bit, f.y & bit, f.z & bit, lane, terms);
        slot = b;
    }
    if (lane != 0) terms = 0.f;
    const float sum = block_sum(terms, scratch);
    if (threadIdx.x == 0) a.partials[slot] = sum;
}

static inline int64_t gs_ws_one(int64_t B, int32_t D) {
    const int64_t nA = (B + teams_per_block(D) - 1) / teams_per_block(D);
    return 2 * align_up(B * (int64_t)D * 4, 256) + align_up((nA + 512) * 4, 256);
}

#ifndef WR_GS_TILES_AT
#define WR_GS_TILES_AT 0
#endif
#ifndef WR_GS_SIDE_AT
#define WR_GS_SIDE_AT 12
#endif
#ifndef WR_GS_NUT
#define WR_GS_NUT 256
#endif
#ifndef WR_GS_NDS
#define WR_GS_NDS 64
#endif
#ifndef WR_GS_NIT
#define WR_GS_NIT 1024
#endif

struct GroupRun {
    TablePair tabs;
    const int32_t *u, *p, *n, *plan;
    int64_t n_triplets, batch_size, plan_words, workspace_bytes, sync_words;
    BatchRange range;
    float lr, *loss_out;
    void *const *events;
    void *workspace;
    uint32_t *sync;
    int n_cu;
    float *grad_slots;
    int64_t n_local_items, global_batch;
    hipStream_t stream;
};

template <int T, int NV, bool FULL>
static int32_t launch_group_steps(const GroupRun &g, const GroupLayout &L, const GpDev &G) {
    const int32_t D = g.tabs.D;
    const int64_t n_batches = g.range.n_batches, global_batch = g.global_batch;
    uint32_t *const sync = g.sync;
    const int64_t B = L.B;
    const int64_t ws_one = gs_ws_one(B, D), zb = align_up(B * (int64_t)D * 4, 256);
    char *ws = reinterpret_cast<char *>(g.workspace);
    float *Zs[2] = {reinterpret_cast<float *>(ws), reinterpret_cast<float *>(ws + ws_one)};
    float *ZUs[2] = {reinterpret_cast<float *>(ws + zb), reinterpret_cast<float *>(ws + ws_one + zb)};
    float *Ps[2] = {reinterpret_cast<float *>(ws + 2 * zb), reinterpret_cast<float *>(ws + ws_one + 2 * zb)};
    constexpr int TEAMS = kBlock / T;
    WR_HIP(hipMemsetAsync(sync, 0, (size_t)(n_batches * kGsStepWords) * 4, g.stream));
    uint32_t *timeout = sync + (g.sync_words - 4);
    int nDS = WR_GS_NDS;
    while (nDS > g.n_cu / 4 && nDS > 1) nDS >>= 1;
    auto batch_of = [&](int64_t b) {
        const int64_t off = b * B;
        const int Bk = (int)batch_len(g.n_triplets, B, b);
        return GsBatch{g.u + off, g.p + off, g.n + off, reinterpret_cast<const uint4 *>(G.flags + b * L.fw * 4),
                       G.ul_row + b * L.R_u * (int64_t)L.cap_u, G.ul_src + b * L.R_u * (int64_t)L.cap_u, G.ucnt + b * L.R_u,
                       G.il_row + b * L.R_i * (int64_t)L.cap_i, G.il_src + b * L.R_i * (int64_t)L.cap_i, G.icnt + b * L.R_i,
                       Bk, L.R_u, L.R_i, L.cap_u, L.cap_i};
    };
    auto ev = [&](int64_t k, int j) { return g.events ? reinterpret_cast<hipEvent_t>(g.events[2 * k + j]) : (hipEvent_t) nullptr; };
    int n_partials_prev = 0;
    for (int64_t k = 0; k <= n_batches; ++k) {
        GsArgs a{};
        a.U = g.tabs.U;
        a.I = g.tabs.I;
        a.D = D;
        a.lr = g.lr;
        a.done = sync + (k < n_batches ? k : 0) * kGsStepWords;
        a.timeout = timeout;
        a.Gs = g.grad_slots;
        a.nL = (int)g.n_local_items;
        const bool have_cur = k < n_batches, have_prev = k > 0;
        if (have_cur) {
            a.cur = batch_of(g.range.first_batch + k);
            a.Z = Zs[k & 1];
            a.ZU = ZUs[k & 1];
            a.partials = Ps[k & 1];
            a.denom = global_batch > 0 ? (float)global_batch : (float)a.cur.B;
            a.nA = (int)((a.cur.B + TEAMS - 1) / TEAMS);
            a.nDS = have_prev ? nDS : 0;
            a.chained = have_prev ? 1 : 0;
        }
        if (have_prev) {
            a.prev = batch_of(g.range.first_batch + k - 1);
            a.Zp = Zs[(k - 1) & 1];
            a.ZUp = ZUs[(k - 1) & 1];
            a.partials_prev = Ps[(k - 1) & 1];
            a.n_partials_prev = n_partials_prev;
            a.denom_prev = global_batch > 0 ? (float)global_batch : (float)a.prev.B;
            a.loss_prev = at_or_null(g.loss_out, k - 1);
            a.nIT = (int)std::min<int64_t>(WR_GS_NIT, (2 * B + kGsTile - 1) / kGsTile + L.R_i);
            a.nUT = (int)std::min<int64_t>(WR_GS_NUT, (B + kGsTile - 1) / kGsTile + L.R_u);
        }
        a.tiles_at = (int)((int64_t)a.nA * WR_GS_TILES_AT / 16);
        a.side_at = std::max(a.tiles_at, (int)((int64_t)a.nA * WR_GS_SIDE_AT / 16));
        const dim3 grid((unsigned)(a.nA + a.nIT + a.nUT + a.nDS));
        hipEvent_t e0 = have_cur ? ev(k, 0) : nullptr, e1 = have_cur ? ev(k, 1) : nullptr;
        if (e0 != nullptr || e1 != nullptr)
            hipExtLaunchKernelGGL((bprmf_group_step<T, NV, FULL>), grid, dim3(kBlock), 0, g.stream, e0, e1, 0, a);
        else
            hipLaunchKernelGGL((bprmf_group_step<T, NV, FULL>), grid, dim3(kBlock), 0, g.stream, a);
        WR_LAUNCH_CHECK("bprmf_group_step");
        n_partials_prev = a.nA + a.nDS;
    }
    return WR_OK;
}

static int32_t check_group_plan(const char *entry, const GroupRun &g, GroupLayout &L) {
    int32_t rc;
    if ((rc = check_whole_lines(entry, whole_lines(g.tabs.U, g.tabs.I, g.tabs.D), g.tabs.D)) != WR_OK) return rc;
    WR_REQUIRE(group_layout(g.n_triplets, g.batch_size, g.tabs.n_users, g.tabs.n_items, L), WR_E_RANGE,
               "group plan not applicable to n=%lld, batch=%lld", (long long)g.n_triplets, (long long)g.batch_size);
    WR_REQUIRE(g.plan_words >= L.total, WR_E_WORKSPACE, "group plan: %lld words < %lld", (long long)g.plan_words, (long long)L.total);
    return WR_OK;
}

static int32_t run_group(const char *entry, GroupRun &g, const GroupLayout &L, int64_t sync_batches) {
    int32_t rc;
    if ((rc = check_workspace(entry, g.workspace, g.workspace_bytes, 2 * gs_ws_one(g.batch_size, g.tabs.D))) != WR_OK) return rc;
    if ((rc = check_sync_words(entry, g.sync, g.sync_words, sync_batches * kGsStepWords + 4)) != WR_OK) return rc;
    if (g.range.n_batches == 0) return WR_OK;
    if (g.n_cu == 0 && (rc = device_cu_count(&g.n_cu)) != WR_OK) return rc;
    const GpDev G = group_dev(const_cast<int32_t *>(g.plan), L);
#define WR_CALL_GS(T_, NV_, FULL_) return launch_group_steps<T_, NV_, FULL_>(g, L, G)
    WR_DISPATCH_D(g.tabs.D, WR_CALL_GS);
#undef WR_CALL_GS
    return WR_OK;
}

}

using namespace wr;

extern "C" {

int64_t wr_group_plan_words(int64_t n_triplets, int64_t batch_size, int64_t n_users, int64_t n_items) {
    GroupLayout L;
    if (!group_layout(n_triplets, batch_size, n_users, n_items, L)) return 0;
    return L.total;
}

int32_t wr_group_plan_layout(int64_t n_triplets, int64_t batch_size, int64_t n_users, int64_t n_items, int64_t *out) {
    WR_REQUIRE(out != nullptr, WR_E_NULL, "out is NULL");
    GroupLayout L;
    WR_REQUIRE(group_layout(n_triplets, batch_size, n_users, n_items, L), WR_E_RANGE,
               "group plan not applicable to n=%lld, batch=%lld", (long long)n_triplets, (long long)batch_size);
    const int64_t v[16] = {L.nb, L.fw, L.R_u, L.R_i, (int64_t)L.mask_u, (int64_t)L.mask_i, L.flags, L.ucnt, L.icnt, L.ul_row,
                           L.ul_src, L.il_row, L.il_src, L.total, L.cap_u, L.cap_i};
    for (int i = 0; i < 16; ++i) out[i] = v[i];
    return WR_OK;
}

int32_t wr_narrow_ids_i64(const int64_t *u, const int64_t *p, const int64_t *n, int32_t *u32, int32_t *p32, int32_t *n32,
                          int64_t count, void *stream_) {
    WR_REQUIRE(u && p && n && u32 && p32 && n32, WR_E_NULL, "index arrays must not be NULL");
    WR_REQUIRE(count >= 0 && count < (int64_t(1) << 40), WR_E_SHAPE, "count out of range");
    if (count == 0) return WR_OK;
    hipLaunchKernelGGL(narrow_ids_kernel, dim3((unsigned)((count + kBlock - 1) / kBlock)), dim3(kBlock), 0,
                       reinterpret_cast<hipStream_t>(stream_), u, p, n, u32, p32, n32, count);
    WR_LAUNCH_CHECK("narrow_ids_kernel");
    return WR_OK;
}

int32_t wr_group_plan_build(const int32_t *u, const int32_t *p, const int32_t *n, int64_t n_triplets, int64_t batch_size,
                            int64_t n_users, int64_t n_items, int32_t *plan, int64_t plan_words, void *stream_) {
    WR_REQUIRE(u && p && n && plan, WR_E_NULL, "index arrays / plan must not be NULL");
    GroupLayout L;
    WR_REQUIRE(group_layout(n_triplets, batch_size, n_users, n_items, L), WR_E_RANGE,
               "group plan not applicable to n=%lld, batch=%lld", (long long)n_triplets, (long long)batch_size);
    WR_REQUIRE(aligned16(plan) && plan_words >= L.total, WR_E_WORKSPACE, "group plan: %lld words < %lld", (long long)plan_words,
               (long long)L.total);
    WR_REQUIRE(L.nb * (L.R_u + L.R_i) < (int64_t(1) << 31), WR_E_SHAPE, "group plan: too many batches in one plan");
    hipStream_t stream = reinterpret_cast<hipStream_t>(stream_);
    WR_HIP(hipMemsetAsync(plan, 0, (size_t)L.zero_words * 4, stream));
    const size_t lds = (size_t)(2 * kGpCap + kGpWords + 3 * L.fw + 4) * 4;
    static bool attr_set = false;
    if (!attr_set) {
        WR_HIP(hipFuncSetAttribute(reinterpret_cast<const void *>(group_plan_kernel), hipFuncAttributeMaxDynamicSharedMemorySize,
                                   (int)((2 * kGpCap + kGpWords + 3 * ((kGpMaxBatch + 31) / 32) + 4) * 4)));
        attr_set = true;
    }
    const GpDev G = group_dev(plan, L);
    hipLaunchKernelGGL(group_plan_kernel, dim3((unsigned)(L.nb * (L.R_u + L.R_i))), dim3(kGpThreads), lds, stream, u, p, n,
                       n_triplets, (int)batch_size, (int)L.nb, (int)n_users, (int)n_items, G);
    WR_LAUNCH_CHECK("group_plan_kernel");
    return WR_OK;
}

int64_t wr_bprmf_group_workspace_bytes(int64_t batch_size, int32_t D) { return 2 * gs_ws_one(batch_size, D); }

int64_t wr_bprmf_group_sync_words(int64_t n_batches) { return n_batches < 0 ? WR_E_SHAPE : (n_batches + 1) * kGsStepWords + 4; }

int32_t wr_bprmf_group_supported(const float *user_tab, const float *item_tab, int32_t D) {
    return (user_tab && item_tab && D >= 4 && D <= 1024 && D % 4 == 0 && whole_lines(user_tab, item_tab, D)) ? 1 : 0;
}

int32_t wr_bprmf_run_sgd_group(float *user_tab, int64_t n_users, float *item_tab, int64_t n_items, int32_t D,
                               const int32_t *u, const int32_t *p, const int32_t *n, int64_t n_triplets, int64_t batch_size,
                               const int32_t *plan, int64_t plan_words, int64_t first_batch, int64_t n_batches, float lr,
                               float *loss_out, void *const *events, void *workspace, int64_t workspace_bytes, int32_t *sync,
                               int64_t sync_words, void *stream) {
    GroupRun g{};
    g.tabs = TablePair{user_tab, item_tab, n_users, n_items, D};
    g.u = u; g.p = p; g.n = n; g.n_triplets = n_triplets; g.batch_size = batch_size;
    g.plan = plan; g.plan_words = plan_words;
    g.range = BatchRange{first_batch, n_batches};
    g.lr = lr; g.loss_out = loss_out; g.events = events;
    g.workspace = workspace; g.workspace_bytes = workspace_bytes;
    g.sync = reinterpret_cast<uint32_t *>(sync); g.sync_words = sync_words;
    g.stream = reinterpret_cast<hipStream_t>(stream);
    int32_t rc;
    GroupLayout L;
    if ((rc = check_tables(g.tabs)) != WR_OK) return rc;
    WR_REQUIRE(u && p && n && plan && sync, WR_E_NULL, "index arrays / plan / sync words must not be NULL");
    if ((rc = check_group_plan("wr_bprmf_run_sgd_group", g, L)) != WR_OK) return rc;
    WR_REQUIRE(first_batch >= 0 && n_batches >= 0 && first_batch + n_batches <= L.nb, WR_E_SHAPE,
               "batches [%lld,%lld) exceed the plan's %lld", (long long)first_batch, (long long)(first_batch + n_batches),
               (long long)L.nb);
    return run_group("wr_bprmf_run_sgd_group", g, L, n_batches + 1);
}

int32_t wr_bprmf_shard_step_group(float *user_shard, int64_t n_user_rows, float *item_ext, int64_t n_ext_rows,
                                  int64_t n_local_items, int32_t D, const int32_t *vu, const int32_t *vp, const int32_t *vn,
                                  int64_t n_triplets, int64_t batch_size, const int32_t *plan, int64_t plan_words, int64_t batch,
                                  int64_t global_batch, float lr, float *grad_slots, float *loss_partial, void *workspace,
                                  int64_t workspace_bytes, int32_t *sync, int64_t sync_words, void *stream) {
    GroupRun g{};
    g.tabs = TablePair{user_shard, item_ext, n_user_rows, n_ext_rows, D};
    g.u = vu; g.p = vp; g.n = vn; g.n_triplets = n_triplets; g.batch_size = batch_size;
    g.plan = plan; g.plan_words = plan_words;
    g.range = BatchRange{batch, 1};
    g.lr = lr; g.loss_out = loss_partial;
    g.workspace = workspace; g.workspace_bytes = workspace_bytes;
    g.sync = reinterpret_cast<uint32_t *>(sync); g.sync_words = sync_words;
    g.n_cu = 256;
    g.grad_slots = grad_slots; g.n_local_items = n_local_items; g.global_batch = global_batch;
    g.stream = reinterpret_cast<hipStream_t>(stream);
    int32_t rc;
    GroupLayout L;
    if ((rc = check_tables(g.tabs, "user_shard", "item_ext")) != WR_OK) return rc;
    WR_REQUIRE(vu && vp && vn && plan && sync && grad_slots, WR_E_NULL, "index arrays / plan / sync words / grad_slots must not be NULL");
    WR_REQUIRE(aligned16(grad_slots), WR_E_ALIGN, "grad_slots is not 16-byte aligned");
    WR_REQUIRE(n_local_items >= 0 && n_local_items <= n_ext_rows, WR_E_SHAPE, "n_local_items %lld outside [0, %lld]",
               (long long)n_local_items, (long long)n_ext_rows);
    if ((rc = check_group_plan("wr_bprmf_shard_step_group", g, L)) != WR_OK) return rc;
    WR_REQUIRE(batch >= 0 && batch < L.nb, WR_E_SHAPE, "batch %lld outside the plan's %lld", (long long)batch, (long long)L.nb);
    WR_REQUIRE(global_batch >= batch_size, WR_E_SHAPE, "global_batch %lld < local batch %lld", (long long)global_batch,
               (long long)batch_size);
    return run_group("wr_bprmf_shard_step_group", g, L, 2);
}

}
```

### whisprrec_amd/hip_ops.py

```python
import ctypes

import torch

from . import abi


def _stream():
    return torch.cuda.current_stream().cuda_stream


def _p(t):
    return None if t is None else t.data_ptr()


def _addr(struct):
    return ctypes.addressof(struct) if struct is not None else None


def _event_handles(events, per_step, count, allow_none):
    if events is None:
        return None
    if len(events) != per_step * count:
        raise ValueError("%s must hold %d events per step" % ("phase_events" if per_step == 4 else "events", per_step))
    handles = []
# ... 403 lines not shown
        if self._want_overlap:
            self._enqueue_overlap_marks()

    def _hot_arrays(self, dev):
        i32 = dict(dtype=torch.int32, device=dev)
        nb = self.n_batches
        sides = []
        for kind in (0, 1):
            if self.arena is not None:
                buf, cp, cr = self.arena.hot_sides[kind]
                m = self.arena.max_batches
                arrs = [buf[:nb * cp], buf[m * cp:m * cp + nb * cp], buf[2 * m * cp:2 * m * cp + nb * cr],
                        buf[2 * m * cp + m * cr:2 * m * cp + m * cr + nb * cr],
                        buf[2 * m * cp + 2 * m * cr:2 * m * cp + 2 * m * cr + nb * cr]]
            else:
                cp, cr = hot_caps(self.batch_size, kind)
                arrs = [torch.empty(nb * cp, **i32), torch.empty(nb * cp, **i32), torch.empty(nb * cr, **i32),
                        torch.empty(nb * cr, **i32), torch.empty(nb * cr, **i32)]
            sides.append((arrs, cp, cr))
        return sides

    def _enqueue_hot_runs(self):
        L = abi.lib()
        counts = self.meta[self.META_HEAD:self.META_HEAD + 4 * self.n_batches]
        for (kind, keys), (arrs, _, _) in zip(((0, self.oc_item), (1, self.tu)), self._sides):
            abi.check(L.wr_bprmf_plan_hot_runs(_p(keys), kind, self.n_triplets, self.batch_size, *[_p(a) for a in arrs],
                                               _p(counts), _stream()), "wr_bprmf_plan_hot_runs")

    def _enqueue_overlap_marks(self):
        o, cb = self.arena.overlap, self._cap_batches
        counts = self.meta[self.META_HEAD + 4 * cb:self.META_HEAD + 5 * cb]
        L = abi.lib()
        fn = L.wr_bprmf_plan_overlap_deferred if getattr(self, "_bitmap_ready", False) else L.wr_bprmf_plan_overlap_marks
        abi.check(fn(_p(self.tu), _p(self.tp), _p(self.tn), self.n_triplets, self.batch_size, self.n_items, None,
                     _p(o["bitmap"]), _p(o["tdef"]), _p(o["def_q"]), o["cap"], _p(counts), _stream()),
                  "wr_bprmf_plan_overlap_marks")

    def _queue_readback(self):
        if self._pinned is not None:
            self._pinned.copy_(self.meta, non_blocking=True)
            self.ready = torch.cuda.Event()
            self.ready.record(self._stream)

    def _read_meta(self):
        if self._pinned is not None:
            self.ready.synchronize()
            return self._pinned
        return self.meta.cpu()

    def finish(self):
        if self._finished:
            return self
        mh = None
        while self._tried in ("fast", "fast+map") or self._want_hot:
            mh = self._read_meta()
            overflow = int(self.arena.meta_np[1]) if self._pinned is not None else int(mh[1])
            if self._tried in ("fast", "fast+map") and overflow != 0:
                if self._builder_arg == "fast":
                    raise abi.WhisprRecHipError("fast plan builder: bucket overflow (skewed ids)")
                self.fast_overflowed = True
                if self._tried == "fast":
                    _FAST_BACKOFF[self._backoff_key] = 32
                with torch.cuda.stream(self._stream):
                    self.meta.zero_()
                    self._build_generic()
                    self._queue_readback()
                mh = None
                continue
            break
        self.meta_host = mh
        if self.builder is None:
            self.builder = self._tried
        if self._want_hot:
            if self._pinned is not None:
                any_hot = bool(self.arena.meta_np[self.META_HEAD:self.META_HEAD + 4 * self.n_batches].any())
            else:
                any_hot = int(mh[self.META_HEAD:self.META_HEAD + 4 * self.n_batches].sum().item()) > 0
            if any_hot:
                self.hot = {"sides": self._sides, "counts_host": mh[self.META_HEAD:self.META_HEAD + 4 * self.n_batches]}
        if self._want_overlap and self.hot is None:
            o, nb, cb = self.arena.overlap, self.n_batches, self._cap_batches
            views = self.arena.views.get((nb, cb))
            if views is None:
                lo = self.META_HEAD + 4 * cb
                views = self.arena.views[(nb, cb)] = (mh[lo:lo + nb], self.arena.meta_np[lo:lo + nb], self.meta[lo:lo + cb])
            dc, dcn, dcd = views
            lo_n, hi_n = (int(dcn.min()), int(dcn.max())) if nb >= 2 else (-1, -1)
            if nb >= 2 and lo_n >= 0:
                self.overlap = {"tdef": o["tdef"], "def_q": o["def_q"], "def_count_host": dc, "cap": o["cap"],
                                "def_count_np": dcn, "fits": hi_n <= o["cap"], "def_count_dev": dcd}
        self._finished = True
        return self

    def hot_struct(self, batch=None):
        self.finish()
        if self.hot is None:
            return None
        k = 0 if batch is None else batch
        vals = []
        for arrs, cp, cr in self.hot["sides"]:
            vals += [arrs[0].data_ptr() + 4 * k * cp, arrs[1].data_ptr() + 4 * k * cp, arrs[2].data_ptr() + 4 * k * cr,
                     arrs[3].data_ptr() + 4 * k * cr, arrs[4].data_ptr() + 4 * k * cr]
        (_, cp0, cr0), (_, cp1, cr1) = self.hot["sides"]
        return abi.HotRuns(*vals, self.hot["counts_host"].data_ptr() + 16 * k, cp0, cr0, cp1, cr1)

    def validate(self):
        if self._unchecked:
            raise abi.WhisprRecHipError("this plan was built with validate=False and keeps no index-range flag")
        self.finish()
        if self.meta_host is None:
            self.meta_host = self._read_meta()
        bad = int(self.arena.meta_np[0]) if self._pinned is not None else int(self.meta_host[0].item())
        if bad != 0:
            raise IndexError("index out of range in batch (user_id >= n_users or item id >= n_items)")

    def batch_len(self, k):
        return min(self.batch_size, self.n_triplets - k * self.batch_size)

    def record_stream(self, stream):
        if self.arena is not None:
            return
        ts = [self.tu, self.tp, self.tn, self.oc_item, self.oc_src, self.meta]
        if self.torig is not None:
            ts.append(self.torig)
        if self._sides is not None:
            for arrs, _, _ in self._sides:
                ts += arrs
        for t in ts:
            t.record_stream(stream)


class GroupArena:

    def __init__(self, device, max_triplets, batch_size, n_users, n_items):
        words = int(abi.lib().wr_group_plan_words(int(max_triplets), int(batch_size), int(n_users), int(n_items)))
        if words <= 0:
            raise abi.WhisprRecHipError("group plan: shape not supported (batch size %d)" % batch_size)
        self.device, self.max_triplets, self.batch_size = device, int(max_triplets), int(batch_size)
        self.n_users, self.n_items = int(n_users), int(n_items)
        self.buf = torch.empty(words, dtype=torch.int32, device=device)
        self.meta_host = torch.zeros(GroupPlan.META, dtype=torch.int32, pin_memory=True)
        self.meta_np = self.meta_host.numpy()
        self.free = None

    def release_after(self, stream):
        self.free = torch.cuda.Event()
        self.free.record(stream)


class GroupPlan:

    META = 16

    def __init__(self, u, p, n, batch_size, n_users, n_items, arena=None, defer=False):
        u, p, n = (_req(t, torch.int32, nm, 1) for t, nm in ((u, "u"), (p, "p"), (n, "n")))
        N = u.numel()
        if not (p.numel() == N and n.numel() == N) or N == 0:
            raise ValueError("u/p/n must have the same non-zero length")
        L = abi.lib()
        self.u, self.p, self.n = u, p, n
        self.n_triplets, self.batch_size = N, int(batch_size)
        self.n_users, self.n_items = int(n_users), int(n_items)
        self.n_batches = (N + self.batch_size - 1) // self.batch_size
        self.words = int(L.wr_group_plan_words(N, self.batch_size, self.n_users, self.n_items))
        if self.words <= 0:
            raise abi.WhisprRecHipError("group plan: shape not supported (batch size %d)" % self.batch_size)
        self.arena = arena
        self._stream = torch.cuda.current_stream(u.device)
        if arena is not None:
            if arena.buf.numel() < self.words or arena.batch_size != self.batch_size or \
                    (arena.n_users, arena.n_items) != (self.n_users, self.n_items):
                raise ValueError("plan does not fit its arena")
            if arena.free is not None:
                self._stream.wait_event(arena.free)
                arena.free = None
            self.buf = arena.buf
            self._pinned = arena.meta_host
        else:
            self.buf = torch.empty(self.words, dtype=torch.int32, device=u.device)
            self._pinned = None
        abi.check(L.wr_group_plan_build(_p(u), _p(p), _p(n), N, self.batch_size, self.n_users, self.n_items, _p(self.buf),
                                        self.buf.numel(), _stream()), "wr_group_plan_build")
        self.ready = None
        if self._pinned is not None:
            self._pinned.copy_(self.buf[:self.META], non_blocking=True)
            self.ready = torch.cuda.Event()
            self.ready.record(self._stream)
        self._finished = False
        self.bad_index = self.overflow = self.long_run = False
        if not defer:
            self.finish()

    def finish(self):
        if self._finished:
            return self
        if self._pinned is not None:
            self.ready.synchronize()
            m = self.arena.meta_np
        else:
            m = self.buf[:self.META].cpu().numpy()
        self.bad_index, self.overflow, self.long_run = bool(m[0]), bool(m[1]), bool(m[2])
        self._finished = True
        return self

    def finish_from(self, meta):
        self.bad_index, self.overflow, self.long_run = bool(meta[0]), bool(meta[1]), bool(meta[2])
        self._finished = True
        return self

    def validate(self):
        self.finish()
        if self.bad_index:
            raise IndexError("index out of range in batch (user_id >= n_users or item id >= n_items)")

    def batch_len(self, k):
        return min(self.batch_size, self.n_triplets - k * self.batch_size)

    def layout(self):
        out = (ctypes.c_int64 * 16)()
        abi.check(abi.lib().wr_group_plan_layout(self.n_triplets, self.batch_size, self.n_users, self.n_items,
                                                 ctypes.addressof(out)), "wr_group_plan_layout")
        keys = ("nb", "fw", "R_u", "R_i", "mask_u", "mask_i", "flags", "ucnt", "icnt", "ul_row", "ul_src", "il_row", "il_src",
                "total", "cap_u", "cap_i")
        return dict(zip(keys, [int(v) for v in out]))

    def decode(self):
        import numpy as np
        self.finish()
        Ly = self.layout()
        w = self.buf[:Ly["total"]].cpu().numpy()
        nb, fw = Ly["nb"], Ly["fw"]
        flags = w[Ly["flags"]:Ly["flags"] + nb * fw * 4].view(np.uint32).reshape(nb, fw, 4).copy()
        out = {"flags": flags, "users": {}, "items": {}, "R_u": Ly["R_u"], "R_i": Ly["R_i"], "meta": w[:self.META].copy()}
        for side, R, cap, co, ro, so in (("users", Ly["R_u"], Ly["cap_u"], "ucnt", "ul_row", "ul_src"),
                                         ("items", Ly["R_i"], Ly["cap_i"], "icnt", "il_row", "il_src")):
            for b in range(nb):
                for r in range(R):
                    c = int(w[Ly[co] + b * R + r])
                    at = (b * R + r) * cap
                    out[side][(b, r)] = (w[Ly[ro] + at:Ly[ro] + at + c].astype(np.int64),
                                         w[Ly[so] + at:Ly[so] + at + c].astype(np.int64))
        return out


_CHAIN_SYNC = {}
_OVERLAP_WS_BYTES = {}


class BprmfTables:

    def __init__(self, user_tab, item_tab):
        self.U = _req(user_tab, torch.float32, "user_tab", 2)
        self.I = _req(item_tab, torch.float32, "item_tab", 2)
        if self.U.shape[1] != self.I.shape[1]:
            raise ValueError("user and item tables must have the same embedding size")
        self.D = self.U.shape[1]
        self.dev = self.U.device
        self.stamp_u = None
        self.stamp_i = None
        self.step_id = 0

    def _stamps(self):
        if self.stamp_u is None:
            self.stamp_u = torch.full((self.U.shape[0],), -1, dtype=torch.int32, device=self.dev)
            self.stamp_i = torch.full((self.I.shape[0],), -1, dtype=torch.int32, device=self.dev)
        return self.stamp_u, self.stamp_i

    def _ws(self, B):
        nbytes = abi.check_size(abi.lib().wr_bprmf_step_workspace_bytes(B, self.D), "wr_bprmf_step_workspace_bytes")
        return workspace(self.dev, "step").get(nbytes)

    def _loss_buf(self, out, count=None):
        return out if out is not None else torch.empty(() if count is None else count, dtype=torch.float32, device=self.dev)

    def _table_head(self):
        return (_p(self.U), self.U.shape[0], _p(self.I), self.I.shape[0], self.D)

    @staticmethod
    def _plan_head(plan):
        return (_p(plan.tu), _p(plan.tp), _p(plan.tn), _p(plan.oc_item), _p(plan.oc_src), plan.n_triplets, plan.batch_size)

    def _plan_ptrs(self, plan, k):
        off = k * plan.batch_size
        return (plan.tu.data_ptr() + 4 * off, plan.tp.data_ptr() + 4 * off, plan.tn.data_ptr() + 4 * off,
                plan.oc_item.data_ptr() + 8 * off, plan.oc_src.data_ptr() + 8 * off, plan.batch_len(k))

    def step_sgd(self, plan, k, lr, l2=0.0, loss_out=None, decay_untouched=True):
        L = abi.lib()
        ws = self._ws(plan.batch_size)
        loss_out = self._loss_buf(loss_out)
        su = si = None
        self.step_id += 1
        if l2 != 0.0:
            su, si = self._stamps()
        hot = plan.hot_struct(k)
        abi.check(L.wr_bprmf_step_sgd(*self._table_head(), *self._plan_ptrs(plan, k), lr, l2, _p(su), _p(si), self.step_id,
                                      _p(loss_out), _addr(hot), _p(ws), ws.numel(), _stream()), "wr_bprmf_step_sgd")
        if l2 != 0.0 and decay_untouched:
            abi.check(L.wr_sgd_decay_untouched(_p(self.U), self.U.shape[0], self.D, _p(su), self.step_id, lr, l2,
                                               _stream()), "wr_sgd_decay_untouched")
            abi.check(L.wr_sgd_decay_untouched(_p(self.I), self.I.shape[0], self.D, _p(si), self.step_id, lr, l2,
                                               _stream()), "wr_sgd_decay_untouched")
        return loss_out

    def run_sgd(self, plan, first, count, lr, losses=None, phase_events=None):
        L = abi.lib()
        ws = self._ws(plan.batch_size)
        losses = self._loss_buf(losses, count)
        hot = plan.hot_struct()
        ev = _event_handles(phase_events, 4, count, True)
        abi.check(L.wr_bprmf_run_sgd(*self._table_head(), *self._plan_head(plan), first, count, lr, _p(losses), _addr(ev),
                                     _addr(hot), _p(ws), ws.numel(), _stream()), "wr_bprmf_run_sgd")
        self.step_id += count
        return losses

    def overlap_workspace(self, batch_size):
        nbytes = _OVERLAP_WS_BYTES.get((batch_size, self.D))
        if nbytes is None:
            nbytes = _OVERLAP_WS_BYTES[(batch_size, self.D)] = 2 * abi.check_size(
                abi.lib().wr_bprmf_step_workspace_bytes(batch_size, self.D), "wr_bprmf_step_workspace_bytes")
        return workspace(self.dev, "step_overlap").get(nbytes)

    def chain_supported(self):
        return bool(abi.lib().wr_bprmf_chain_supported(_p(self.U), _p(self.I), self.D))

    CHAIN_SYNC_STEPS = 256

    def _chain_sync(self, count):
        key = (str(self.dev), torch.cuda.current_stream(self.dev).cuda_stream)
        bufs = _CHAIN_SYNC.setdefault(key, [])
        if bufs and count <= self.CHAIN_SYNC_STEPS:
            return bufs[-1]
        if not bufs or bufs[-1].numel() < int(abi.lib().wr_bprmf_chain_sync_words(count)):
            words = int(abi.lib().wr_bprmf_chain_sync_words(max(count, self.CHAIN_SYNC_STEPS)))
            bufs.append(torch.zeros(words, dtype=torch.int32, device=self.dev))
        return bufs[-1]

    def sticky_words(self):
        sid = torch.cuda.current_stream(self.dev).cuda_stream
        return [buf[-4:-3] for key, bufs in _CHAIN_SYNC.items() if key[0] == str(self.dev) and key[1] == sid for buf in bufs]

    def check_chain(self):
        for key, bufs in _CHAIN_SYNC.items():
            if key[0] != str(self.dev):
                continue
            for buf in bufs:
                if int(buf[-4].item()) != 0:
                    raise abi.WhisprRecHipError("chained step launch: a wait for the item tiles expired — the tables are "
                                                "not valid")

    def run_sgd_chain(self, plan, first, count, lr, losses=None, phase_events=None, ws=None, def_limit=None):
        L = abi.lib()
        o = plan.overlap
        if ws is None:
            ws = self.overlap_workspace(plan.batch_size)
        losses = self._loss_buf(losses, count)
        ev = _event_handles(phase_events, 4, count, True)
        sync = self._chain_sync(count)
        abi.check(L.wr_bprmf_run_sgd_chain(*self._table_head(), *self._plan_head(plan), first, count, lr, _p(losses),
                                           _p(o["tdef"]), _p(o["def_q"]), o["def_count_host"].data_ptr(), o["cap"],
                                           o["cap"] if def_limit is None else int(def_limit), _addr(ev), _p(ws), ws.numel(),
                                           _p(sync), sync.numel(), _stream()), "wr_bprmf_run_sgd_chain")
        self.step_id += count
        return losses

    def group_supported(self):
        return bool(abi.lib().wr_bprmf_group_supported(_p(self.U), _p(self.I), self.D))

    def _group_sync(self, count):
        key = (str(self.dev), torch.cuda.current_stream(self.dev).cuda_stream, "group")
        bufs = _CHAIN_SYNC.setdefault(key, [])
        need = int(abi.lib().wr_bprmf_group_sync_words(count))
        if not bufs or bufs[-1].numel() < need:
            words = int(abi.lib().wr_bprmf_group_sync_words(max(count, self.CHAIN_SYNC_STEPS)))
            bufs.append(torch.zeros(words, dtype=torch.int32, device=self.dev))
        return bufs[-1]

    def run_sgd_group(self, gplan, first, count, lr, losses=None, events=None):
        L = abi.lib()
        nbytes = abi.check_size(L.wr_bprmf_group_workspace_bytes(gplan.batch_size, self.D), "wr_bprmf_group_workspace_bytes")
        ws = workspace(self.dev, "group_step").get(nbytes)
        losses = self._loss_buf(losses, count)
        ev = _event_handles(events, 2, count, False)
        sync = self._group_sync(count)
        abi.check(L.wr_bprmf_run_sgd_group(*self._table_head(), _p(gplan.u), _p(gplan.p), _p(gplan.n), gplan.n_triplets,
                                           gplan.batch_size, _p(gplan.buf), gplan.buf.numel(), first, count, lr, _p(losses),
                                           _addr(ev), _p(ws), ws.numel(), _p(sync), sync.numel(), _stream()),
                  "wr_bprmf_run_sgd_group")
        self.step_id += count
        return losses

    def grads(self, plan, k, grad_u, grad_i, loss_out=None, stamps=True):
        L = abi.lib()
        ws = self._ws(plan.batch_size)
        su, si = self._stamps() if stamps else (None, None)
        loss_out = self._loss_buf(loss_out)
        self.step_id += 1
        hot = plan.hot_struct(k)
        abi.check(L.wr_bprmf_grads(*self._table_head(), *self._plan_ptrs(plan, k), _p(grad_u), _p(grad_i), _p(su), _p(si),
                                   self.step_id, _p(loss_out), _addr(hot), _p(ws), ws.numel(), _stream()), "wr_bprmf_grads")
        return loss_out, self.step_id


PAIR_SET_MIN_PAIRS = 1 << 20


def pair_set(clicked_ptr, clicked_idx, n_users):
    _req(clicked_ptr, torch.int64, "clicked_ptr", 1)
    _req(clicked_idx, torch.int32, "clicked_idx", 1)
    L = abi.lib()
    cap = abi.check_size(L.wr_pairset_capacity(int(clicked_idx.numel())), "wr_pairset_capacity")
    table = torch.empty(cap, dtype=torch.int64, device=clicked_ptr.device)
    err = torch.zeros(1, dtype=torch.int32, device=clicked_ptr.device)
    abi.check(L.wr_pairset_build(_p(clicked_ptr), _p(clicked_idx), int(n_users), _p(table), cap, _p(err), _stream()),
              "wr_pairset_build")
    if int(err.item()) != 0:
        raise abi.WhisprRecHipError("pair set: table too small")
    return table


def sample_negatives(users, n_users, n_items, clicked_ptr, clicked_idx, seed, epoch, pairs=None):
    if users.dtype not in (torch.int64, torch.int32):
        raise TypeError("users must be int64 or int32")
    users = _req(users.contiguous(), users.dtype, "users", 1)
    if pairs is None:
        _req(clicked_ptr, torch.int64, "clicked_ptr", 1)
        _req(clicked_idx, torch.int32, "clicked_idx", 1)
    neg = torch.empty_like(users)
    err = torch.zeros(1, dtype=torch.int32, device=users.device)
    L = abi.lib()
    if pairs is not None:
        fn = L.wr_sample_negatives_set_i64 if users.dtype == torch.int64 else L.wr_sample_negatives_set_i32
        abi.check(fn(_p(users), users.numel(), n_users, n_items, _p(_req(pairs, torch.int64, "pairs", 1)), pairs.numel(), seed,
                     epoch, _p(neg), _p(err), _stream()), "wr_sample_negatives_set")
        return neg, err
    fn = L.wr_sample_negatives_i64 if users.dtype == torch.int64 else L.wr_sample_negatives_i32
    abi.check(fn(_p(users), users.numel(), n_users, n_items, _p(clicked_ptr), _p(clicked_idx), seed, epoch, _p(neg), _p(err),
                 _stream()), "wr_sample_negatives")
    return neg, err


def epoch_shuffle(cols, seed, epoch, want_order=False):
    cols = list(cols)
    if not 1 <= len(cols) <= 3:
        raise ValueError("one to three columns")
    dt = cols[0].dtype
    if dt not in (torch.int64, torch.int32):
        raise TypeError("columns must be int64 or int32")
    n = cols[0].numel()
    cols = [_req(c.contiguous(), dt, "column", 1) for c in cols]
    if any(c.numel() != n for c in cols):
        raise ValueError("columns must have the same length")
    outs = [torch.empty_like(c) for c in cols]
    order = torch.empty(n, dtype=torch.int64, device=cols[0].device) if want_order else None
    pad = [None] * (3 - len(cols))
    fn = abi.lib().wr_epoch_shuffle_i64 if dt == torch.int64 else abi.lib().wr_epoch_shuffle_i32
    abi.check(fn(*[_p(c) for c in cols + pad], n, int(seed), int(epoch), *[_p(o) for o in outs + pad], _p(order), _stream()),
              "wr_epoch_shuffle")
    return (outs, order) if want_order else outs


class EpochPrep:

    def __init__(self, users, items, n_users, n_items, clicked_ptr, clicked_idx, seed, epoch, want_order=False, pairs=None,
                 packed=None):
        if users.dtype not in (torch.int64, torch.int32) or items.dtype != users.dtype:
            raise TypeError("users / items must both be int64 or int32")
        self.users = _req(users.contiguous(), users.dtype, "users", 1)
        self.items = _req(items.contiguous(), users.dtype, "items", 1)
        if self.items.numel() != self.users.numel():
            raise ValueError("users / items must have the same length")
        if pairs is None:
            _req(clicked_ptr, torch.int64, "clicked_ptr", 1)
            _req(clicked_idx, torch.int32, "clicked_idx", 1)
        self.ptr, self.idx = clicked_ptr, clicked_idx
        self.pairs = None if pairs is None else _req(pairs, torch.int64, "pairs", 1)
        self.packed = None
        if packed is not None and pairs is not None:
            self.packed = _req(packed, torch.int64, "packed", 1)
            if self.packed.numel() != self.users.numel():
                raise ValueError("packed rows: one word per interaction")
        self.n, self.n_users, self.n_items = users.numel(), int(n_users), int(n_items)
        self.seed, self.epoch = int(seed), int(epoch)
        self.cols = [torch.empty_like(self.users) for _ in range(3)]
        self.order = torch.empty(self.n, dtype=torch.int64, device=users.device) if want_order else None
        self.err = torch.zeros(1, dtype=torch.int32, device=users.device)
        self.filled = 0

    def fill(self, lo, hi):
        lo, hi = int(lo), min(int(hi), self.n)
        if hi <= lo:
            return
        es = self.users.element_size()
        L = abi.lib()
        tail = (self.seed, self.epoch, lo, hi - lo, self.cols[0].data_ptr() + es * lo, self.cols[1].data_ptr() + es * lo,
                self.cols[2].data_ptr() + es * lo, None if self.order is None else self.order.data_ptr() + 8 * lo,
                _p(self.err), _stream())
        if self.packed is not None:
            fn = L.wr_epoch_prepare_range_packed_i64 if self.users.dtype == torch.int64 else L.wr_epoch_prepare_range_packed_i32
            abi.check(fn(_p(self.packed), self.n, self.n_users, self.n_items, _p(self.pairs), self.pairs.numel(), *tail),
                      "wr_epoch_prepare_range_packed")
        elif self.pairs is not None:
            fn = L.wr_epoch_prepare_range_set_i64 if self.users.dtype == torch.int64 else L.wr_epoch_prepare_range_set_i32
            abi.check(fn(_p(self.users), _p(self.items), self.n, self.n_users, self.n_items, _p(self.pairs), self.pairs.numel(),
                         *tail), "wr_epoch_prepare_range_set")
        else:
            fn = L.wr_epoch_prepare_range_i64 if self.users.dtype == torch.int64 else L.wr_epoch_prepare_range_i32
            abi.check(fn(_p(self.users), _p(self.items), self.n, self.n_users, self.n_items, _p(self.ptr), _p(self.idx), *tail),
                      "wr_epoch_prepare_range")
        self.filled = max(self.filled, hi)

    def check(self):
        if int(self.err.item()) == 1:
            raise IndexError("user id out of range in the training frame")


def pack_rows(users, items):
    return ((users.to(torch.int64) << 32) | items.to(torch.int64)).contiguous()


def clicked_csr_from_pairs(users, items, n_users, n_items):
    key = torch.unique(users.to(torch.int64) * int(n_items) + items.to(torch.int64))
    uu = torch.div(key, int(n_items), rounding_mode="floor")
    ptr = torch.zeros(n_users + 1, dtype=torch.int64, device=users.device)
    ptr[1:] = torch.cumsum(torch.bincount(uu, minlength=n_users), 0)
    return ptr, (key - uu * int(n_items)).to(torch.int32)


def clicked_csr(train_clicked_set, n_users, device):
    import numpy as np
    ptr = np.zeros(n_users + 1, np.int64)
    chunks = []
    for uu in range(n_users):
        items = train_clicked_set.get(uu, ())
        ptr[uu + 1] = ptr[uu] + len(items)
        if len(items):
            chunks.append(np.sort(np.fromiter(items, dtype=np.int32, count=len(items))))
    idx = np.concatenate(chunks) if chunks else np.zeros(1, np.int32)
    return torch.from_numpy(ptr).to(device), torch.from_numpy(idx).to(device)


LDS_PER_WORKGROUP = 160 * 1024

# ... 518 lines not shown
    def backward(ctx, grad_out):
        history, item_weight = ctx.saved_tensors[:2]
        rest = list(ctx.saved_tensors[2:])
        pos_weight = rest.pop(0) if ctx.has_pos else None
        W1, b1, W2, b2 = rest
        g_hp, gW1, gb1, gW2, gb2, gpos = interest_pool_bwd(item_weight, pos_weight, history, W1, b1, W2, b2, grad_out.contiguous())
        g_item = torch.zeros_like(item_weight)
        ids = history.reshape(-1).clamp(0, item_weight.shape[0] - 1)
        scatter_add_rows(g_item, ids, g_hp.view(-1, g_hp.shape[2]), padding_idx=0)
        return g_item, gpos, gW1, gb1, gW2, gb2, None, None


def interest_pool(item_weight, pos_weight, history, W1, b1, W2, b2, err_word=None):
    return _InterestPool.apply(item_weight, pos_weight, W1, b1, W2, b2, history, err_word)


def sgd_dense(tab, grad, lr, l2=0.0, stamp=None, step_id=0):
    abi.check(abi.lib().wr_sgd_dense(_p(_req(tab, torch.float32, "tab", 2)), tab.shape[0], tab.shape[1],
                                     _p(_req(grad, torch.float32, "grad", 2)), _p(stamp), step_id, lr, l2, _stream()),
              "wr_sgd_dense")


def adam_dense(tab, exp_avg, exp_avg_sq, grad, adam_step, lr, l2=0.0, beta1=0.9, beta2=0.999, eps=1e-8, stamp=None,
               step_id=0):
    for t, nm in ((tab, "tab"), (exp_avg, "exp_avg"), (exp_avg_sq, "exp_avg_sq"), (grad, "grad")):
        _req(t, torch.float32, nm, 2)
    abi.check(abi.lib().wr_adam_dense(_p(tab), _p(exp_avg), _p(exp_avg_sq), tab.shape[0], tab.shape[1], _p(grad),
                                      _p(stamp), step_id, adam_step, lr, l2, beta1, beta2, eps, _stream()),
              "wr_adam_dense")


def _join_views(ts):
    if len(ts) == 1:
        return ts[0]
    a = ts[0]
    adjacent, end = a.is_contiguous(), a.storage_offset() + a.numel()
    for b in ts[1:]:
        adjacent = adjacent and b.is_contiguous() and b.dtype == a.dtype and \
            b.untyped_storage().data_ptr() == a.untyped_storage().data_ptr() and b.storage_offset() == end
        end += b.numel()
    if adjacent:
        return torch.as_strided(a, (end - a.storage_offset(),), (1,), a.storage_offset())
    return torch.cat(ts)


class PipelinedSgd:

    PREFETCH_AFTER_TRIPLETS = 0
    PLAN_TRIPLETS = 1 << 22
    GROUP_MIN_ROWS_PER_TRIPLET = 12
    GROUP_MIN_BATCH = 4096

    CHAIN_MIN_BATCH = 8192
    CHAIN_MIN_ITEMS_PER_TRIPLET = 6

    def __init__(self, chunk=64, min_triplets=None, chain=True, inline_plan=False, group=True):
        import sys
        self.ops = sys.modules[__name__]
        self.chunk = int(chunk)
        self.chain = bool(chain)
        self.group = bool(group)
        self.inline_plan = inline_plan
        self.stats = {"plain_calls": 0, "chain_calls": 0, "group_calls": 0, "group_fallbacks": 0}
        self._garenas = {}
        if min_triplets is not None:
            self.PLAN_TRIPLETS = int(min_triplets)
        self.plan_stream = None
        self._arenas = {}

    def chunk_batches(self, batch_size):
        return max(self.chunk, self.PLAN_TRIPLETS // max(int(batch_size), 1))

    def _arena_pair(self, device, B, nb_total, overlap_items):
        cap = min(self.chunk_batches(B), max(int(nb_total), 1)) * B
        key = (str(device), B, int(overlap_items))
        pair = self._arenas.get(key)
        if pair is None or pair[0].max_triplets < cap:
            pair = [self.ops.PlanArena(device, cap, B, overlap_items=overlap_items) for _ in range(2)]
            self._arenas[key] = pair
        return pair

    def _garena_pair(self, device, B, nb_total, n_users, n_items):
        cap = min(self.chunk_batches(B), max(int(nb_total), 1)) * B
        key = (str(device), B, int(n_users), int(n_items))
        pair = self._garenas.get(key)
        if pair is None or pair[0].max_triplets < cap:
            pair = [self.ops.GroupArena(device, cap, B, n_users, n_items) for _ in range(2)]
            self._garenas[key] = pair
        return pair

    def plan(self, U, segments, batch, first_chunk=None, lr=None, prep=None, runner=None):
        if self.plan_stream is None:
            self.plan_stream = side_stream(U.device)
        B = int(batch)
        segs, first = [], 0
        for k, (rows, u, p, n) in enumerate(segments):
            nb = (u.numel() + B - 1) // B
            if u.numel() % B != 0 and any(s[1].numel() for s in segments[k + 1:]):
                raise ValueError("only the last segment may end with a short batch")
            segs.append({"tabs": self.ops.BprmfTables(U, rows) if nb else None, "nb": nb, "first": first})
            first += nb
        live = [s for s in segments if s[1].numel()]
        u_all, p_all, n_all = (_join_views([s[j] for s in live]) for j in (1, 2, 3))
        n_items = max([s[0].shape[0] for s in live] or [1])
        main = torch.cuda.current_stream(U.device)
        use_chain = self.chain and (runner is None or getattr(runner, "wants_chain_marks", False)) and \
            B >= self.CHAIN_MIN_BATCH and first >= 2 and \
            min([s[0].shape[0] for s in live] or [0]) >= self.CHAIN_MIN_ITEMS_PER_TRIPLET * B and \
            all(sg["tabs"].chain_supported() for sg in segs if sg["tabs"] is not None)
        min_rows = min([U.shape[0]] + [s[0].shape[0] for s in live])
        use_group = self.group and runner is None and len(live) == 1 and first >= 2 and \
            self.GROUP_MIN_BATCH <= B <= 131072 and u_all.dtype in (torch.int32, torch.int64) and \
            min_rows >= self.GROUP_MIN_ROWS_PER_TRIPLET * B and \
            all(sg["tabs"].group_supported() for sg in segs if sg["tabs"] is not None)
        garenas = self._garena_pair(U.device, B, first, U.shape[0], n_items) if use_group else None
        arenas = None if use_group else self._arena_pair(U.device, B, first, n_items if use_chain else 0)
        for a in (arenas or []) + (garenas or []):
            a.release_after(main)
        h = {"segs": segs, "B": B, "u": u_all, "p": p_all, "n": n_all, "nb": first, "n_users": U.shape[0], "n_items": n_items,
             "at": 0, "tag": 0, "next": None, "cur": None, "map": None, "arenas": arenas, "pos": 0,
             "group": use_group, "garenas": garenas, "device": U.device,
             "ids32": [torch.empty(u_all.numel(), dtype=torch.int32, device=U.device) for _ in range(3)]
                      if use_group and u_all.dtype == torch.int64 else None,
             "chain": use_chain, "prep": prep, "runner": runner, "inline": bool(self.inline_plan),
             "lead": [int(c) for c in (first_chunk if isinstance(first_chunk, (list, tuple)) else [first_chunk or 0]) if c]}
        self.plan_stream.wait_stream(main)
        self._prefetch(h)
        return h

    def _build_stream(self, h):
        return torch.cuda.current_stream(h["u"].device) if h["inline"] else self.plan_stream

    def _prefetch(self, h):
        if h["at"] >= h["nb"]:
            h["next"] = None
            return
        first, B = h["at"], h["B"]
        c = min(self.chunk_batches(B), h["nb"] - first)
        if h["lead"]:
            c = min(c, h["lead"].pop(0))
        h["at"] += c
        lo, hi = first * B, min(h["u"].numel(), (first + c) * B)
        with torch.cuda.stream(self._build_stream(h)):
            bmap = h["map"] if h["map"] else None
            if h["prep"] is not None:
                h["prep"].fill(lo, hi)
            if h["group"]:
                cols = (h["u"], h["p"], h["n"])
                if h["ids32"] is not None:
                    abi.check(abi.lib().wr_narrow_ids_i64(*[_p(c[lo:hi]) for c in cols], *[_p(c[lo:hi]) for c in h["ids32"]],
                                                          hi - lo, _stream()), "wr_narrow_ids_i64")
                    cols = h["ids32"]
                plan = self.ops.GroupPlan(cols[0][lo:hi], cols[1][lo:hi], cols[2][lo:hi], B, h["n_users"], h["n_items"],
                                          arena=h["garenas"][h["tag"]], defer=True)
                h["tag"] ^= 1
                h["next"] = (first, plan)
                return
            if h["arenas"] is None:
                h["arenas"] = self._arena_pair(h["device"], B, h["nb"], h["n_items"] if h["chain"] else 0)
            plan = self.ops.BatchPlan(h["u"][lo:hi], h["p"][lo:hi], h["n"][lo:hi], B, h["n_users"], h["n_items"],
                                      validate=False, ws_tag="rot%d" % h["tag"], bucket_map=bmap, arena=h["arenas"][h["tag"]],
                                      defer=True, overlap=h["chain"])
        h["tag"] ^= 1
        h["next"] = (first, plan)

    STICKY_MSG = "a wait inside a step launch expired (hand-off between the workgroups of one launch): the tables are not " \
                 "valid — do not save or evaluate them; restart the run"

    def _queue_sticky(self, h, tabs, main):
        words = tabs.sticky_words()
        if not words:
            return
        pin = h.get("sticky_pin")
        if pin is None or pin.numel() < 2 * len(words):
            pin = h["sticky_pin"] = torch.zeros(2 * max(len(words), 4), dtype=torch.int32, pin_memory=True)
        half = pin.numel() // 2
        off = half * (h.get("sticky_tag", 0) & 1)
        h["sticky_tag"] = h.get("sticky_tag", 0) + 1
        for j, wd in enumerate(words):
            pin[off + j:off + j + 1].copy_(wd, non_blocking=True)
        ev = torch.cuda.Event()
        ev.record(main)
        self._check_sticky(h)
        h["sticky_pending"] = (ev, pin[off:off + len(words)])

    def _check_sticky(self, h):
        pend = h.pop("sticky_pending", None)
        if pend is not None:
            pend[0].synchronize()
            if bool(pend[1].numpy().any()):
                raise abi.WhisprRecHipError(self.STICKY_MSG)

    def _take_next(self, h, pos, main):
        self._check_sticky(h)
        if h["next"] is None:
            self._prefetch(h)
        cur = h["next"]
        assert cur is not None and cur[0] == pos, "steps must be run in order"
        plan = cur[1]
        plan.validate()
        if isinstance(plan, GroupPlan):
            if plan.overflow or plan.long_run:
                h["group"] = False
                self.stats["group_fallbacks"] += 1
                if h["next"] is not None and h["next"][0] != cur[0]:
                    raise AssertionError("plan pipeline out of step")
                if plan.overflow:
                    first, B = cur[0], h["B"]
                    lo, hi = first * B, first * B + plan.n_triplets
                    plan.arena.release_after(main)
                    if h["arenas"] is None:
                        h["arenas"] = self._arena_pair(h["device"], B, h["nb"], h["n_items"] if h["chain"] else 0)
                    with torch.cuda.stream(self._build_stream(h)):
                        plan = self.ops.BatchPlan(h["u"][lo:hi], h["p"][lo:hi], h["n"][lo:hi], B, h["n_users"], h["n_items"],
                                                  validate=False, ws_tag="rot%d" % h["tag"], arena=h["arenas"][h["tag"]],
                                                  defer=True, overlap=h["chain"])
                    h["tag"] ^= 1
                    plan.validate()
                    cur = (first, plan)
            main.wait_event(plan.ready)
            h["cur"], h["next"] = cur, None
            return cur
        main.wait_event(plan.ready)
        if plan.fast_overflowed:
            if plan._mapped():
                h["map"] = False
            elif h["map"] is None:
                with torch.cuda.stream(self._build_stream(h)):
                    src = (h["prep"].users, h["prep"].items) if h["prep"] is not None else (h["u"], h["p"])
                    h["map"] = self.ops.BucketMap(src[0], src[1], h["n_users"], h["n_items"], h["B"])
        if h["chain"] and plan.hot is not None:
            h["chain"] = False
        if h["chain"] and plan.hot is None and plan.overlap is not None and not plan.overlap["fits"]:
            dcn = plan.overlap["def_count_np"]
            if int((dcn[1:] > plan.overlap["cap"]).sum()) * 2 > plan.n_batches - 1:
                h["chain"] = False
        h["cur"], h["next"] = cur, None
        return cur

    def _run_span(self, h, sg, pos, end, lr, losses, loss_off):
        main = torch.cuda.current_stream(sg["tabs"].U.device)
        while pos < end:
            cur = h["cur"]
            if cur is None or pos >= cur[0] + cur[1].n_batches:
                cur = self._take_next(h, pos, main)
            base, plan = cur
            c = min(end, base + plan.n_batches) - pos
            if h["inline"] and h["next"] is None and h["at"] < h["nb"]:
                mid = base + plan.n_batches // 2
                if pos >= mid:
                    self._prefetch(h)
                else:
                    c = min(c, mid - pos)
            elif self.PREFETCH_AFTER_TRIPLETS > 0 and h["next"] is None and h["at"] < h["nb"] and \
                    c > (self.PREFETCH_AFTER_TRIPLETS + h["B"] - 1) // h["B"]:
                c = (self.PREFETCH_AFTER_TRIPLETS + h["B"] - 1) // h["B"]
            if isinstance(plan, GroupPlan):
                sg["tabs"].run_sgd_group(plan, pos - base, c, lr, losses=losses[loss_off:loss_off + c])
                self.stats["group_calls"] += 1
            elif h["runner"] is not None:
                h["runner"](plan, pos - base, c, losses[loss_off:loss_off + c])
                self.stats["plain_calls"] += 1
            elif h["chain"] and plan.overlap is not None and c >= 2:
                sg["tabs"].run_sgd_chain(plan, pos - base, c, lr, losses=losses[loss_off:loss_off + c])
                self.stats["chain_calls"] += 1
            else:
                sg["tabs"].run_sgd(plan, pos - base, c, lr, losses=losses[loss_off:loss_off + c])
                self.stats["plain_calls"] += 1
            pos += c
            loss_off += c
            if pos >= base + plan.n_batches:
                plan.arena.release_after(main)
                self._queue_sticky(h, sg["tabs"], main)
            if h["next"] is None and not h["inline"]:
                self._prefetch(h)
        h["pos"] = pos

    def run(self, handle, seg, lr, losses):
        sg = handle["segs"][seg]
        if sg["nb"] == 0:
            return
        self._run_span(handle, sg, sg["first"], sg["first"] + sg["nb"], lr, losses, 0)
        if seg == len(handle["segs"]) - 1:
            self._check_sticky(handle)

    def run_steps(self, handle, count, lr, losses):
        assert len(handle["segs"]) == 1, "run_steps: single-segment handles"
        sg = handle["segs"][0]
        pos = handle["pos"]
        if pos + count > sg["nb"]:
            raise ValueError("run_steps: %d steps asked, %d left" % (count, sg["nb"] - pos))
        self._run_span(handle, sg, pos, pos + count, lr, losses, 0)


class LazyOptimizerState:

    FOLD_MAX_GAP = 40

    MAX_LAG = 64
    LAG_MIN_GAP = 64

    def __init__(self, tabs, name, lr, l2, betas=(0.9, 0.999), eps=1e-8, fold=None, max_lag=None):
        self.chain, self.chain_calls = True, 0
        if name not in ("SGD", "Adam"):
            raise ValueError(name)
        self.tabs, self.name, self.lr, self.l2, self.betas, self.eps = tabs, name, float(lr), float(l2), betas, float(eps)
        self.fold = fold if fold is None else bool(fold)
        self.max_lag = max_lag if max_lag is None else int(max_lag)
        self._sweep_pos = (ctypes.c_int64 * 2)(0, 0)
        dev = tabs.dev
        self.t = 0
        self.flushed_at = 0
        self.last_u = torch.zeros(tabs.U.shape[0], dtype=torch.int32, device=dev)
        self.last_i = torch.zeros(tabs.I.shape[0], dtype=torch.int32, device=dev)
        if name == "Adam":
            z = torch.zeros_like
            self.m_u, self.v_u, self.m_i, self.v_i = z(tabs.U), z(tabs.U), z(tabs.I), z(tabs.I)
            self.consts = None
            self._grow_consts(4096)

    def _folds(self, plan):
        if self.fold is None:
            gap = max(self.tabs.U.shape[0], self.tabs.I.shape[0]) / float(max(plan.batch_size, 1))
            return gap <= self.FOLD_MAX_GAP
        return self.fold

    def _adam_state(self):
        return (_p(self.m_u), _p(self.v_u), _p(self.m_i), _p(self.v_i), _p(self.last_u), _p(self.last_i))

    def _grow_consts(self, n):
        host = torch.empty(2 * n, dtype=torch.float32)
        abi.check(abi.lib().wr_adam_consts(0, n, self.lr, self.betas[0], self.betas[1], host.data_ptr()), "wr_adam_consts")
        self.consts = host.to(self.tabs.dev)
        self.n_consts = n

    def _adam_rows(self, tab, m, v, last, keys_ptr, n_keys, grad):
        abi.check(abi.lib().wr_adam_rows_lazy(_p(tab), _p(m), _p(v), _p(last), tab.shape[0], tab.shape[1], keys_ptr, n_keys,
                                              _p(grad), self.t, _p(self.consts), self.n_consts, self.l2, self.betas[0],
                                              self.betas[1], self.eps, _stream()), "wr_adam_rows_lazy")

    def step(self, plan, k, loss_out=None):
        tabs = self.tabs
        if _auto_lag(self, plan) > 0 and not (self.name == "Adam" and self._folds(plan)):
            out = self.run(plan, k, 1, losses=None if loss_out is None else loss_out.reshape(1))
            return out.reshape(()) if loss_out is None else loss_out
        self.t += 1
        batch = tabs._plan_ptrs(plan, k)
        tu, oi, B = batch[0], batch[3], batch[5]
        if self.name == "Adam":
            if self.t >= self.n_consts:
                self._grow_consts(2 * self.n_consts)
            hot = plan.hot_struct(k)
            folded = self._folds(plan) and hot is None
            if not folded:
                self._adam_rows(tabs.U, self.m_u, self.v_u, self.last_u, tu, B, None)
                self._adam_rows(tabs.I, self.m_i, self.v_i, self.last_i, oi, 2 * B, None)
            loss_out = tabs._loss_buf(loss_out)
            ws = tabs._ws(plan.batch_size)
            head = (*tabs._table_head(), *self._adam_state(), *batch, self.t, self.lr)
            tail = (self.l2, self.betas[0], self.betas[1], self.eps, _p(loss_out))
            if folded:
                abi.check(abi.lib().wr_bprmf_step_adam_folded(*head, _p(self.consts), self.n_consts, *tail, _p(ws), ws.numel(),
                                                              _stream()), "wr_bprmf_step_adam_folded")
            else:
                abi.check(abi.lib().wr_bprmf_step_adam(*head, *tail, _addr(hot), _p(ws), ws.numel(), _stream()),
                          "wr_bprmf_step_adam")
            tabs.step_id += 1
            return loss_out
        L = abi.lib()
        for tab, last, keys, n in ((tabs.U, self.last_u, tu, B), (tabs.I, self.last_i, oi, 2 * B)):
            abi.check(L.wr_sgd_rows_lazy(_p(tab), _p(last), tab.shape[0], tab.shape[1], keys, n, self.t, self.lr, self.l2,
                                         _stream()), "wr_sgd_rows_lazy")
        return tabs.step_sgd(plan, k, self.lr, self.l2, loss_out=loss_out, decay_untouched=False)

    def run(self, plan, first, count, losses=None):
        tabs, L = self.tabs, abi.lib()
        losses = tabs._loss_buf(losses, count)
        ws = tabs._ws(plan.batch_size)
        su, si = tabs._stamps()
        hot = plan.hot_struct()
        t0 = self.t + 1
        lag = _auto_lag(self, plan)
        if self.name == "Adam":
            while self.t + count >= self.n_consts:
                self._grow_consts(2 * self.n_consts)
            head = (*tabs._table_head(), *self._adam_state(), *tabs._plan_head(plan), first, count, t0, self.lr,
                    _p(self.consts), self.n_consts, self.l2, self.betas[0], self.betas[1], self.eps, _p(losses), _addr(hot))
            o = getattr(plan, "overlap", None)
            if self._folds(plan) and self.chain and o is not None and hot is None and count >= 2 and tabs.chain_supported():
                ws2 = tabs.overlap_workspace(plan.batch_size)
                sync = tabs._chain_sync(count)
                abi.check(L.wr_bprmf_run_adam_folded_chain(*head[:-1], _p(o["tdef"]), _p(o["def_q"]),
                                                           o["def_count_host"].data_ptr(), o["cap"], o["cap"], _p(ws2),
                                                           ws2.numel(), _p(sync), sync.numel(), _stream()),
                          "wr_bprmf_run_adam_folded_chain")
                self.chain_calls += 1
            elif self._folds(plan):
                abi.check(L.wr_bprmf_run_adam_folded(*head, _p(ws), ws.numel(), _stream()), "wr_bprmf_run_adam_folded")
            elif lag > 0:
                abi.check(L.wr_bprmf_run_adam_lazy_bounded(*head, lag, _addr(self._sweep_pos), _p(ws), ws.numel(), _stream()),
                          "wr_bprmf_run_adam_lazy_bounded")
            else:
                abi.check(L.wr_bprmf_run_adam_lazy(*head, _p(ws), ws.numel(), _stream()), "wr_bprmf_run_adam_lazy")
        else:
            head = (*tabs._table_head(), _p(self.last_u), _p(self.last_i), _p(su), _p(si), tabs.step_id + 1,
                    *tabs._plan_head(plan), first, count, t0, self.lr, self.l2, _p(losses), _addr(hot))
            if lag > 0:
                abi.check(L.wr_bprmf_run_sgd_lazy_bounded(*head, lag, _addr(self._sweep_pos), _p(ws), ws.numel(), _stream()),
                          "wr_bprmf_run_sgd_lazy_bounded")
            else:
                abi.check(L.wr_bprmf_run_sgd_lazy(*head, _p(ws), ws.numel(), _stream()), "wr_bprmf_run_sgd_lazy")
        self.t += count
        tabs.step_id += count
        return losses

    def flush(self):
        if self.flushed_at == self.t:
            return
        L, tabs = abi.lib(), self.tabs
        if self.name == "Adam":
            for tab, m, v, last in ((tabs.U, self.m_u, self.v_u, self.last_u), (tabs.I, self.m_i, self.v_i, self.last_i)):
                abi.check(L.wr_adam_catchup_all(_p(tab), _p(m), _p(v), _p(last), *tab.shape, self.t, _p(self.consts),
                                                self.n_consts, self.l2, self.betas[0], self.betas[1], self.eps, _stream()),
                          "wr_adam_catchup_all")
        else:
            for tab, last in ((tabs.U, self.last_u), (tabs.I, self.last_i)):
# ... 496 lines not shown
```

Measured before the change: 2.584 billion triplets/s.

## Carry open group-step batch across plan chunks to keep step chain unbroken

The group-step launcher can now leave the last batch of a chunk open and pass its state (plan pointers, loss slot, parity, sync slot) to the next call. The next chunk's first kernel then finishes the previous batch while it starts its own, so the pipeline no longer drains at each chunk boundary. The plan builder gains a 'lead' mode that computes the cross-batch flags for the first batch of a new chunk from the previous chunk's tail. Arena release and sticky-word checks move to a side stream gated by events. This adds considerable bookkeeping and carries correctness risk around workspace parity, sync slot reuse and freeing buffers early.

```diff
diff --git a/include/whisprrec_hip.h b/include/whisprrec_hip.h
--- a/include/whisprrec_hip.h
+++ b/include/whisprrec_hip.h
@@ -181,6 +181,24 @@
                                const int32_t *plan, int64_t plan_words, int64_t first_batch, int64_t n_batches, float lr,
                                float *loss_out, void *const *events, void *workspace, int64_t workspace_bytes, int32_t *sync,
                                int64_t sync_words, void *stream);
+
+typedef struct wr_group_carry {
+    const int32_t *u, *p, *n, *plan;
+    int64_t plan_words, n_triplets;
+    int64_t batch;
+    float *loss_slot;
+    int32_t parity, n_partials;
+    int32_t *sync;
+    int64_t sync_slot;
+} wr_group_carry;
+int32_t wr_group_plan_build_after(const int32_t *u, const int32_t *p, const int32_t *n, int64_t n_triplets, int64_t batch_size,
+                                  int64_t n_users, int64_t n_items, int32_t *plan, int64_t plan_words, void *stream);
+int32_t wr_bprmf_run_sgd_group_stream(float *user_tab, int64_t n_users, float *item_tab, int64_t n_items, int32_t D,
+                                      const int32_t *u, const int32_t *p, const int32_t *n, int64_t n_triplets,
+                                      int64_t batch_size, const int32_t *plan, int64_t plan_words, int64_t first_batch,
+                                      int64_t n_batches, float lr, float *loss_out, void *const *events, void *workspace,
+                                      int64_t workspace_bytes, int32_t *sync, int64_t sync_words, const wr_group_carry *carry_in,
+                                      wr_group_carry *carry_out, int32_t close, void *carried_read, void *stream);
 
 int32_t wr_bprmf_plan_overlap_marks(const int32_t *tu, const int32_t *tp, const int32_t *tn, int64_t n_triplets,
                                     int64_t batch_size, int64_t n_items, const int32_t *prev_bitmap, int32_t *bitmap,
diff --git a/whisprrec_amd/abi.py b/whisprrec_amd/abi.py
--- a/whisprrec_amd/abi.py
+++ b/whisprrec_amd/abi.py
@@ -86,6 +86,10 @@
     "wr_bprmf_group_supported": (c_i32, [c_vp, c_vp, c_i32]),
     "wr_bprmf_run_sgd_group": (c_i32, [c_vp, c_i64, c_vp, c_i64, c_i32, c_vp, c_vp, c_vp, c_i64, c_i64, c_vp, c_i64, c_i64,
                                        c_i64, c_f32, c_vp, c_vp, c_vp, c_i64, c_vp, c_i64, c_vp]),
+    "wr_group_plan_build_after": (c_i32, [c_vp, c_vp, c_vp, c_i64, c_i64, c_i64, c_i64, c_vp, c_i64, c_vp]),
+    "wr_bprmf_run_sgd_group_stream": (c_i32, [c_vp, c_i64, c_vp, c_i64, c_i32, c_vp, c_vp, c_vp, c_i64, c_i64, c_vp, c_i64,
+                                              c_i64, c_i64, c_f32, c_vp, c_vp, c_vp, c_i64, c_vp, c_i64, c_vp, c_vp, c_i32,
+                                              c_vp, c_vp]),
     "wr_bprmf_plan_overlap_deferred": (c_i32, [c_vp, c_vp, c_vp, c_i64, c_i64, c_i64, c_vp, c_vp, c_vp, c_vp, c_i64, c_vp,
                                                c_vp]),
     "wr_bprmf_plan_fast_marks_supported": (c_i32, [c_i64, c_i64, c_i64, c_i64]),
@@ -230,6 +234,12 @@
                 ("n_tiles", c_i64)]
 
 
+class GroupCarry(ctypes.Structure):
+    _fields_ = [("u", c_vp), ("p", c_vp), ("n", c_vp), ("plan", c_vp), ("plan_words", c_i64), ("n_triplets", c_i64),
+                ("batch", c_i64), ("loss_slot", c_vp), ("parity", c_i32), ("n_partials", c_i32), ("sync", c_vp),
+                ("sync_slot", c_i64)]
+
+
 class BucketSide(ctypes.Structure):
     _fields_ = [("n_buckets", c_i32), ("row_bucket", c_vp), ("bucket_start", c_vp), ("bucket_rows", c_vp), ("bucket_sub", c_vp)]
 
diff --git a/whisprrec_amd/csrc/wr_group.hip b/whisprrec_amd/csrc/wr_group.hip
--- a/whisprrec_amd/csrc/wr_group.hip
+++ b/whisprrec_amd/csrc/wr_group.hip
@@ -107,7 +107,7 @@
 
 __global__ __launch_bounds__(kGpThreads) void group_plan_kernel(const int *__restrict__ u, const int *__restrict__ p,
                                                                  const int *__restrict__ n, int64_t n_total, int B, int nb,
-                                                                 int n_users, int n_items, GpDev L) {
+                                                                 int n_users, int n_items, GpDev L, int lead) {
     extern __shared__ __attribute__((aligned(16))) unsigned gp_lds[];
     unsigned *seen = gp_lds;
     unsigned long long *keys = reinterpret_cast<unsigned long long *>(gp_lds);
@@ -116,7 +116,8 @@
     int &n_list = *reinterpret_cast<int *>(f2 + L.fw);
     const int per = L.R_u + L.R_i;
     const unsigned lb = xcd_contiguous_id(blockIdx.x, gridDim.x);
-    const int b = (int)(lb / (unsigned)per), rr = (int)(lb % (unsigned)per);
+    const int b = (int)(lb / (unsigned)per) - lead, rr = (int)(lb % (unsigned)per);
+    const bool lead_wg = b < 0;
     const bool item = rr >= L.R_u;
     const unsigned r = (unsigned)(item ? rr - L.R_u : rr);
     const int64_t base = (int64_t)b * B;
@@ -169,40 +170,43 @@
             if (several(row)) atomicOr(&f2[t >> 5], 1u << (t & 31));
         };
         if (item) {
-            gp_scan(p + base, Bb, [&](int row, int t) {
-                if (several(row)) {
-                    atomicOr(&f0[t >> 5], 1u << (t & 31));
-                    append(row, (unsigned)t << 1);
-                }
-            });
-            gp_scan(n + base, Bb, [&](int row, int t) {
-                if (several(row)) {
-                    atomicOr(&f1[t >> 5], 1u << (t & 31));
-                    append(row, ((unsigned)t << 1) | 1u);
-                }
-            });
+            if (!lead_wg) {
+                gp_scan(p + base, Bb, [&](int row, int t) {
+                    if (several(row)) {
+                        atomicOr(&f0[t >> 5], 1u << (t & 31));
+                        append(row, (unsigned)t << 1);
+                    }
+                });
+                gp_scan(n + base, Bb, [&](int row, int t) {
+                    if (several(row)) {
+                        atomicOr(&f1[t >> 5], 1u << (t & 31));
+                        append(row, ((unsigned)t << 1) | 1u);
+                    }
+                });
+            }
             gp_scan(p + nbase, Bn, defer);
             gp_scan(n + nbase, Bn, defer);
         } else {
-            gp_scan(u + base, Bb, [&](int row, int t) {
-                if (several(row)) {
-                    atomicOr(&f0[t >> 5], 1u << (t & 31));
-                    append(row, (unsigned)t << 1);
-                }
-            });
+            if (!lead_wg)
+                gp_scan(u + base, Bb, [&](int row, int t) {
+                    if (several(row)) {
+                        atomicOr(&f0[t >> 5], 1u << (t & 31));
+                        append(row, (unsigned)t << 1);
+                    }
+                });
             gp_scan(u + nbase, Bn, defer);
         }
     }
     __syncthreads();
     if (!(WR_GP_DBG & 4)) {
-        unsigned *fb = L.flags + (int64_t)b * L.fw * 4;
+        unsigned *fb = L.flags + (int64_t)(lead_wg ? 0 : b) * L.fw * 4, *fn = L.flags + (int64_t)(b + 1) * L.fw * 4;
         for (int w = threadIdx.x; w < L.fw; w += kGpThreads) {
             if (f0[w]) __hip_atomic_fetch_or(fb + 4 * w + (item ? 1 : 0), f0[w], __ATOMIC_RELAXED, __HIP_MEMORY_SCOPE_AGENT);
             if (item && f1[w]) __hip_atomic_fetch_or(fb + 4 * w + 2, f1[w], __ATOMIC_RELAXED, __HIP_MEMORY_SCOPE_AGENT);
-            if (f2[w])
-                __hip_atomic_fetch_or(fb + 4 * (L.fw + w) + 3, f2[w], __ATOMIC_RELAXED, __HIP_MEMORY_SCOPE_AGENT);
-        }
-    }
+            if (f2[w]) __hip_atomic_fetch_or(fn + 4 * w + 3, f2[w], __ATOMIC_RELAXED, __HIP_MEMORY_SCOPE_AGENT);
+        }
+    }
+    if (lead_wg) return;
     const int cap = item ? L.cap_i : L.cap_u, R = item ? L.R_i : L.R_u;
     int m = n_list;
     if (m > cap) {
@@ -708,7 +712,19 @@
     float *grad_slots;
     int64_t n_local_items, global_batch;
     hipStream_t stream;
+    const wr_group_carry *carry_in;
+    wr_group_carry *carry_out;
+    hipEvent_t carried_read;
 };
+
+static inline GsBatch gs_batch(const int32_t *u, const int32_t *p, const int32_t *n, int64_t n_triplets, const GroupLayout &L,
+                               const GpDev &G, int64_t b) {
+    const int64_t off = b * L.B;
+    return GsBatch{u + off, p + off, n + off, reinterpret_cast<const uint4 *>(G.flags + b * L.fw * 4),
+                   G.ul_row + b * L.R_u * (int64_t)L.cap_u, G.ul_src + b * L.R_u * (int64_t)L.cap_u, G.ucnt + b * L.R_u,
+                   G.il_row + b * L.R_i * (int64_t)L.cap_i, G.il_src + b * L.R_i * (int64_t)L.cap_i, G.icnt + b * L.R_i,
+                   (int)batch_len(n_triplets, L.B, b), L.R_u, L.R_i, L.cap_u, L.cap_i};
+}
 
 template <int T, int NV, bool FULL>
 static int32_t launch_group_steps(const GroupRun &g, const GroupLayout &L, const GpDev &G) {
@@ -722,49 +738,64 @@
     float *ZUs[2] = {reinterpret_cast<float *>(ws + zb), reinterpret_cast<float *>(ws + ws_one + zb)};
     float *Ps[2] = {reinterpret_cast<float *>(ws + 2 * zb), reinterpret_cast<float *>(ws + ws_one + 2 * zb)};
     constexpr int TEAMS = kBlock / T;
-    WR_HIP(hipMemsetAsync(sync, 0, (size_t)(n_batches * kGsStepWords) * 4, g.stream));
     uint32_t *timeout = sync + (g.sync_words - 4);
     int nDS = WR_GS_NDS;
     while (nDS > g.n_cu / 4 && nDS > 1) nDS >>= 1;
-    auto batch_of = [&](int64_t b) {
-        const int64_t off = b * B;
-        const int Bk = (int)batch_len(g.n_triplets, B, b);
-        return GsBatch{g.u + off, g.p + off, g.n + off, reinterpret_cast<const uint4 *>(G.flags + b * L.fw * 4),
-                       G.ul_row + b * L.R_u * (int64_t)L.cap_u, G.ul_src + b * L.R_u * (int64_t)L.cap_u, G.ucnt + b * L.R_u,
-                       G.il_row + b * L.R_i * (int64_t)L.cap_i, G.il_src + b * L.R_i * (int64_t)L.cap_i, G.icnt + b * L.R_i,
-                       Bk, L.R_u, L.R_i, L.cap_u, L.cap_i};
-    };
+    auto batch_of = [&](int64_t b) { return gs_batch(g.u, g.p, g.n, g.n_triplets, L, G, b); };
     auto ev = [&](int64_t k, int j) { return g.events ? reinterpret_cast<hipEvent_t>(g.events[2 * k + j]) : (hipEvent_t) nullptr; };
+    const wr_group_carry *const ci = g.carry_in;
+    const int par = ci ? (ci->parity ^ 1) : 0;
+    GsBatch carried{};
+    float *carried_loss = nullptr;
     int n_partials_prev = 0;
-    for (int64_t k = 0; k <= n_batches; ++k) {
+    if (ci) {
+        GroupLayout Lc;
+        group_layout(ci->n_triplets, B, g.tabs.n_users, g.tabs.n_items, Lc);
+        carried = gs_batch(ci->u, ci->p, ci->n, ci->n_triplets, Lc, group_dev(const_cast<int32_t *>(ci->plan), Lc), ci->batch);
+        carried_loss = ci->loss_slot;
+        n_partials_prev = ci->n_partials;
+    }
+    int64_t slot0 = 0;
+    if (ci != nullptr || g.carry_out != nullptr) {
+        const int64_t slots = (g.sync_words - 4) / kGsStepWords;
+        if (ci != nullptr && ci->sync == reinterpret_cast<int32_t *>(sync) && ci->sync_slot >= 0 && ci->sync_slot + n_batches <= slots)
+            slot0 = ci->sync_slot;
+        else if (n_batches > 0)
+            WR_HIP(hipMemsetAsync(sync, 0, (size_t)(slots * kGsStepWords) * 4, g.stream));
+    } else if (n_batches > 0) {
+        WR_HIP(hipMemsetAsync(sync, 0, (size_t)(n_batches * kGsStepWords) * 4, g.stream));
+    }
+    const int64_t n_launches = n_batches + (g.carry_out ? 0 : 1);
+    for (int64_t k = 0; k < n_launches; ++k) {
         GsArgs a{};
         a.U = g.tabs.U;
         a.I = g.tabs.I;
         a.D = D;
         a.lr = g.lr;
-        a.done = sync + (k < n_batches ? k : 0) * kGsStepWords;
+        a.done = sync + (k < n_batches ? slot0 + k : 0) * kGsStepWords;
         a.timeout = timeout;
         a.Gs = g.grad_slots;
         a.nL = (int)g.n_local_items;
-        const bool have_cur = k < n_batches, have_prev = k > 0;
+        const bool have_cur = k < n_batches, have_prev = k > 0 || ci != nullptr;
+        if (!have_cur && !have_prev) break;
         if (have_cur) {
             a.cur = batch_of(g.range.first_batch + k);
-            a.Z = Zs[k & 1];
-            a.ZU = ZUs[k & 1];
-            a.partials = Ps[k & 1];
+            a.Z = Zs[(par + k) & 1];
+            a.ZU = ZUs[(par + k) & 1];
+            a.partials = Ps[(par + k) & 1];
             a.denom = global_batch > 0 ? (float)global_batch : (float)a.cur.B;
             a.nA = (int)((a.cur.B + TEAMS - 1) / TEAMS);
             a.nDS = have_prev ? nDS : 0;
             a.chained = have_prev ? 1 : 0;
         }
         if (have_prev) {
-            a.prev = batch_of(g.range.first_batch + k - 1);
-            a.Zp = Zs[(k - 1) & 1];
-            a.ZUp = ZUs[(k - 1) & 1];
-            a.partials_prev = Ps[(k - 1) & 1];
+            a.prev = k > 0 ? batch_of(g.range.first_batch + k - 1) : carried;
+            a.Zp = Zs[(par + k + 1) & 1];
+            a.ZUp = ZUs[(par + k + 1) & 1];
+            a.partials_prev = Ps[(par + k + 1) & 1];
             a.n_partials_prev = n_partials_prev;
             a.denom_prev = global_batch > 0 ? (float)global_batch : (float)a.prev.B;
-            a.loss_prev = at_or_null(g.loss_out, k - 1);
+            a.loss_prev = k > 0 ? at_or_null(g.loss_out, k - 1) : carried_loss;
             a.nIT = (int)std::min<int64_t>(WR_GS_NIT, (2 * B + kGsTile - 1) / kGsTile + L.R_i);
             a.nUT = (int)std::min<int64_t>(WR_GS_NUT, (B + kGsTile - 1) / kGsTile + L.R_u);
         }
@@ -772,13 +803,23 @@
         a.side_at = std::max(a.tiles_at, (int)((int64_t)a.nA * WR_GS_SIDE_AT / 16));
         const dim3 grid((unsigned)(a.nA + a.nIT + a.nUT + a.nDS));
         hipEvent_t e0 = have_cur ? ev(k, 0) : nullptr, e1 = have_cur ? ev(k, 1) : nullptr;
+        bool record_behind = false;
+        if (k == 0 && g.carried_read != nullptr) {
+            if (e1 == nullptr) e1 = g.carried_read;
+            else record_behind = true;
+        }
         if (e0 != nullptr || e1 != nullptr)
             hipExtLaunchKernelGGL((bprmf_group_step<T, NV, FULL>), grid, dim3(kBlock), 0, g.stream, e0, e1, 0, a);
         else
             hipLaunchKernelGGL((bprmf_group_step<T, NV, FULL>), grid, dim3(kBlock), 0, g.stream, a);
         WR_LAUNCH_CHECK("bprmf_group_step");
         n_partials_prev = a.nA + a.nDS;
-    }
+        if (record_behind) WR_HIP(hipEventRecord(g.carried_read, g.stream));
+    }
+    if (g.carry_out)
+        *g.carry_out = wr_group_carry{g.u, g.p, g.n, g.plan, g.plan_words, g.n_triplets, g.range.first_batch + n_batches - 1,
+                                      at_or_null(g.loss_out, n_batches - 1), (int32_t)((par + n_batches - 1) & 1), n_partials_prev,
+                                      reinterpret_cast<int32_t *>(sync), slot0 + n_batches};
     return WR_OK;
 }
 
@@ -795,7 +836,7 @@
     int32_t rc;
     if ((rc = check_workspace(entry, g.workspace, g.workspace_bytes, 2 * gs_ws_one(g.batch_size, g.tabs.D))) != WR_OK) return rc;
     if ((rc = check_sync_words(entry, g.sync, g.sync_words, sync_batches * kGsStepWords + 4)) != WR_OK) return rc;
-    if (g.range.n_batches == 0) return WR_OK;
+    if (g.range.n_batches == 0 && g.carry_in == nullptr) return WR_OK;
     if (g.n_cu == 0 && (rc = device_cu_count(&g.n_cu)) != WR_OK) return rc;
     const GpDev G = group_dev(const_cast<int32_t *>(g.plan), L);
 #define WR_CALL_GS(T_, NV_, FULL_) return launch_group_steps<T_, NV_, FULL_>(g, L, G)
@@ -838,15 +879,15 @@
     return WR_OK;
 }
 
-int32_t wr_group_plan_build(const int32_t *u, const int32_t *p, const int32_t *n, int64_t n_triplets, int64_t batch_size,
-                            int64_t n_users, int64_t n_items, int32_t *plan, int64_t plan_words, void *stream_) {
+static int32_t build_group_plan(const int32_t *u, const int32_t *p, const int32_t *n, int64_t n_triplets, int64_t batch_size,
+                                int64_t n_users, int64_t n_items, int32_t *plan, int64_t plan_words, void *stream_, int lead) {
     WR_REQUIRE(u && p && n && plan, WR_E_NULL, "index arrays / plan must not be NULL");
     GroupLayout L;
     WR_REQUIRE(group_layout(n_triplets, batch_size, n_users, n_items, L), WR_E_RANGE,
                "group plan not applicable to n=%lld, batch=%lld", (long long)n_triplets, (long long)batch_size);
     WR_REQUIRE(aligned16(plan) && plan_words >= L.total, WR_E_WORKSPACE, "group plan: %lld words < %lld", (long long)plan_words,
                (long long)L.total);
-    WR_REQUIRE(L.nb * (L.R_u + L.R_i) < (int64_t(1) << 31), WR_E_SHAPE, "group plan: too many batches in one plan");
+    WR_REQUIRE((L.nb + lead) * (L.R_u + L.R_i) < (int64_t(1) << 31), WR_E_SHAPE, "group plan: too many batches in one plan");
     hipStream_t stream = reinterpret_cast<hipStream_t>(stream_);
     WR_HIP(hipMemsetAsync(plan, 0, (size_t)L.zero_words * 4, stream));
     const size_t lds = (size_t)(2 * kGpCap + kGpWords + 3 * L.fw + 4) * 4;
@@ -857,12 +898,22 @@
         attr_set = true;
     }
     const GpDev G = group_dev(plan, L);
-    hipLaunchKernelGGL(group_plan_kernel, dim3((unsigned)(L.nb * (L.R_u + L.R_i))), dim3(kGpThreads), lds, stream, u, p, n,
-                       n_triplets, (int)batch_size, (int)L.nb, (int)n_users, (int)n_items, G);
+    hipLaunchKernelGGL(group_plan_kernel, dim3((unsigned)((L.nb + lead) * (L.R_u + L.R_i))), dim3(kGpThreads), lds, stream, u, p, n,
+                       n_triplets, (int)batch_size, (int)L.nb, (int)n_users, (int)n_items, G, lead);
     WR_LAUNCH_CHECK("group_plan_kernel");
     return WR_OK;
 }
 
+int32_t wr_group_plan_build(const int32_t *u, const int32_t *p, const int32_t *n, int64_t n_triplets, int64_t batch_size,
+                            int64_t n_users, int64_t n_items, int32_t *plan, int64_t plan_words, void *stream) {
+    return build_group_plan(u, p, n, n_triplets, batch_size, n_users, n_items, plan, plan_words, stream, 0);
+}
+
+int32_t wr_group_plan_build_after(const int32_t *u, const int32_t *p, const int32_t *n, int64_t n_triplets, int64_t batch_size,
+                                  int64_t n_users, int64_t n_items, int32_t *plan, int64_t plan_words, void *stream) {
+    return build_group_plan(u, p, n, n_triplets, batch_size, n_users, n_items, plan, plan_words, stream, 1);
+}
+
 int64_t wr_bprmf_group_workspace_bytes(int64_t batch_size, int32_t D) { return 2 * gs_ws_one(batch_size, D); }
 
 int64_t wr_bprmf_group_sync_words(int64_t n_batches) { return n_batches < 0 ? WR_E_SHAPE : (n_batches + 1) * kGsStepWords + 4; }
@@ -871,11 +922,12 @@
     return (user_tab && item_tab && D >= 4 && D <= 1024 && D % 4 == 0 && whole_lines(user_tab, item_tab, D)) ? 1 : 0;
 }
 
-int32_t wr_bprmf_run_sgd_group(float *user_tab, int64_t n_users, float *item_tab, int64_t n_items, int32_t D,
-                               const int32_t *u, const int32_t *p, const int32_t *n, int64_t n_triplets, int64_t batch_size,
-                               const int32_t *plan, int64_t plan_words, int64_t first_batch, int64_t n_batches, float lr,
-                               float *loss_out, void *const *events, void *workspace, int64_t workspace_bytes, int32_t *sync,
-                               int64_t sync_words, void *stream) {
+static int32_t group_steps_entry(const char *entry, float *user_tab, int64_t n_users, float *item_tab, int64_t n_items, int32_t D,
+                                 const int32_t *u, const int32_t *p, const int32_t *n, int64_t n_triplets, int64_t batch_size,
+                                 const int32_t *plan, int64_t plan_words, int64_t first_batch, int64_t n_batches, float lr,
+                                 float *loss_out, void *const *events, void *workspace, int64_t workspace_bytes, int32_t *sync,
+                                 int64_t sync_words, const wr_group_carry *carry_in, wr_group_carry *carry_out,
+                                 void *carried_read, void *stream) {
     GroupRun g{};
     g.tabs = TablePair{user_tab, item_tab, n_users, n_items, D};
     g.u = u; g.p = p; g.n = n; g.n_triplets = n_triplets; g.batch_size = batch_size;
@@ -884,16 +936,54 @@
     g.lr = lr; g.loss_out = loss_out; g.events = events;
     g.workspace = workspace; g.workspace_bytes = workspace_bytes;
     g.sync = reinterpret_cast<uint32_t *>(sync); g.sync_words = sync_words;
+    g.carry_in = carry_in; g.carry_out = carry_out; g.carried_read = reinterpret_cast<hipEvent_t>(carried_read);
     g.stream = reinterpret_cast<hipStream_t>(stream);
     int32_t rc;
     GroupLayout L;
     if ((rc = check_tables(g.tabs)) != WR_OK) return rc;
     WR_REQUIRE(u && p && n && plan && sync, WR_E_NULL, "index arrays / plan / sync words must not be NULL");
-    if ((rc = check_group_plan("wr_bprmf_run_sgd_group", g, L)) != WR_OK) return rc;
+    if ((rc = check_group_plan(entry, g, L)) != WR_OK) return rc;
     WR_REQUIRE(first_batch >= 0 && n_batches >= 0 && first_batch + n_batches <= L.nb, WR_E_SHAPE,
                "batches [%lld,%lld) exceed the plan's %lld", (long long)first_batch, (long long)(first_batch + n_batches),
                (long long)L.nb);
-    return run_group("wr_bprmf_run_sgd_group", g, L, n_batches + 1);
+    WR_REQUIRE(carry_out == nullptr || n_batches >= 1, WR_E_SHAPE, "%s: no batch to leave open", entry);
+    if (carry_in != nullptr) {
+        const wr_group_carry &c = *carry_in;
+        WR_REQUIRE(c.u && c.p && c.n && c.plan, WR_E_NULL, "carried batch: index arrays / plan must not be NULL");
+        GroupLayout Lc;
+        WR_REQUIRE(group_layout(c.n_triplets, batch_size, n_users, n_items, Lc), WR_E_RANGE,
+                   "group plan not applicable to n=%lld, batch=%lld", (long long)c.n_triplets, (long long)batch_size);
+        WR_REQUIRE(aligned16(c.plan) && c.plan_words >= Lc.total, WR_E_WORKSPACE, "group plan: %lld words < %lld",
+                   (long long)c.plan_words, (long long)Lc.total);
+        WR_REQUIRE(c.batch >= 0 && c.batch < Lc.nb, WR_E_SHAPE, "carried batch %lld outside its plan's %lld", (long long)c.batch,
+                   (long long)Lc.nb);
+        const int64_t nA = (batch_size + teams_per_block(D) - 1) / teams_per_block(D);
+        WR_REQUIRE((c.parity == 0 || c.parity == 1) && c.n_partials >= 0 && c.n_partials <= nA + WR_GS_NDS, WR_E_SHAPE,
+                   "carried batch: slot %d / %d loss partials out of range", (int)c.parity, (int)c.n_partials);
+    }
+    return run_group(entry, g, L, n_batches + 1);
+}
+
+int32_t wr_bprmf_run_sgd_group(float *user_tab, int64_t n_users, float *item_tab, int64_t n_items, int32_t D,
+                               const int32_t *u, const int32_t *p, const int32_t *n, int64_t n_triplets, int64_t batch_size,
+                               const int32_t *plan, int64_t plan_words, int64_t first_batch, int64_t n_batches, float lr,
+                               float *loss_out, void *const *events, void *workspace, int64_t workspace_bytes, int32_t *sync,
+                               int64_t sync_words, void *stream) {
+    return group_steps_entry("wr_bprmf_run_sgd_group", user_tab, n_users, item_tab, n_items, D, u, p, n, n_triplets, batch_size,
+                             plan, plan_words, first_batch, n_batches, lr, loss_out, events, workspace, workspace_bytes, sync,
+                             sync_words, nullptr, nullptr, nullptr, stream);
+}
+
+int32_t wr_bprmf_run_sgd_group_stream(float *user_tab, int64_t n_users, float *item_tab, int64_t n_items, int32_t D,
+                                      const int32_t *u, const int32_t *p, const int32_t *n, int64_t n_triplets,
+                                      int64_t batch_size, const int32_t *plan, int64_t plan_words, int64_t first_batch,
+                                      int64_t n_batches, float lr, float *loss_out, void *const *events, void *workspace,
+                                      int64_t workspace_bytes, int32_t *sync, int64_t sync_words, const wr_group_carry *carry_in,
+                                      wr_group_carry *carry_out, int32_t close, void *carried_read, void *stream) {
+    WR_REQUIRE(close != 0 || carry_out != nullptr, WR_E_NULL, "wr_bprmf_run_sgd_group_stream: carry_out is NULL and close is 0");
+    return group_steps_entry("wr_bprmf_run_sgd_group_stream", user_tab, n_users, item_tab, n_items, D, u, p, n, n_triplets,
+                             batch_size, plan, plan_words, first_batch, n_batches, lr, loss_out, events, workspace,
+                             workspace_bytes, sync, sync_words, carry_in, close ? nullptr : carry_out, carried_read, stream);
 }
 
 int32_t wr_bprmf_shard_step_group(float *user_shard, int64_t n_user_rows, float *item_ext, int64_t n_ext_rows,
diff --git a/whisprrec_amd/hip_ops.py b/whisprrec_amd/hip_ops.py
--- a/whisprrec_amd/hip_ops.py
+++ b/whisprrec_amd/hip_ops.py
@@ -579,11 +579,14 @@
 
     META = 16
 
-    def __init__(self, u, p, n, batch_size, n_users, n_items, arena=None, defer=False):
+    def __init__(self, u, p, n, batch_size, n_users, n_items, arena=None, defer=False, after=False):
         u, p, n = (_req(t, torch.int32, nm, 1) for t, nm in ((u, "u"), (p, "p"), (n, "n")))
         N = u.numel()
         if not (p.numel() == N and n.numel() == N) or N == 0:
             raise ValueError("u/p/n must have the same non-zero length")
+        if after and min(t.storage_offset() for t in (u, p, n)) < int(batch_size):
+            raise ValueError("after=True: u/p/n must be views with a whole batch in front of them")
+        self.after = bool(after)
         L = abi.lib()
         self.u, self.p, self.n = u, p, n
         self.n_triplets, self.batch_size = N, int(batch_size)
@@ -606,8 +609,9 @@
         else:
             self.buf = torch.empty(self.words, dtype=torch.int32, device=u.device)
             self._pinned = None
-        abi.check(L.wr_group_plan_build(_p(u), _p(p), _p(n), N, self.batch_size, self.n_users, self.n_items, _p(self.buf),
-                                        self.buf.numel(), _stream()), "wr_group_plan_build")
+        build = L.wr_group_plan_build_after if self.after else L.wr_group_plan_build
+        abi.check(build(_p(u), _p(p), _p(n), N, self.batch_size, self.n_users, self.n_items, _p(self.buf), self.buf.numel(),
+                        _stream()), "wr_group_plan_build_after" if self.after else "wr_group_plan_build")
         self.ready = None
         if self._pinned is not None:
             self._pinned.copy_(self.buf[:self.META], non_blocking=True)
@@ -816,6 +820,30 @@
                   "wr_bprmf_run_sgd_group")
         self.step_id += count
         return losses
+
+    def run_sgd_group_stream(self, gplan, first, count, lr, losses=None, carry=None, close=True, carried_read=None):
+        L = abi.lib()
+        nbytes = abi.check_size(L.wr_bprmf_group_workspace_bytes(gplan.batch_size, self.D), "wr_bprmf_group_workspace_bytes")
+        ws = workspace(self.dev, "group_step").get(nbytes)
+        if count > 0 or losses is None:
+            losses = self._loss_buf(losses, count)
+        sync = self._group_sync(count)
+        if carry is not None and carry.ws_ptr != ws.data_ptr():
+            raise abi.WhisprRecHipError("group step stream: the workspace moved while a batch was open")
+        out = None if close else abi.GroupCarry()
+        if carried_read is not None and not carried_read.cuda_event:
+            raise ValueError("carried_read must have been recorded once")
+        abi.check(L.wr_bprmf_run_sgd_group_stream(*self._table_head(), _p(gplan.u), _p(gplan.p), _p(gplan.n), gplan.n_triplets,
+                                                  gplan.batch_size, _p(gplan.buf), gplan.buf.numel(), first, count, lr,
+                                                  _p(losses) if count > 0 else None, None, _p(ws), ws.numel(), _p(sync),
+                                                  sync.numel(), _addr(carry), _addr(out), 1 if close else 0,
+                                                  carried_read.cuda_event if carried_read is not None else None, _stream()),
+                  "wr_bprmf_run_sgd_group_stream")
+        self.step_id += count
+        if out is not None:
+            out.ws_ptr = ws.data_ptr()
+            out.keep = (gplan, losses)
+        return losses, out
 
     def grads(self, plan, k, grad_u, grad_i, loss_out=None, stamps=True):
         L = abi.lib()
@@ -1640,7 +1668,7 @@
                                                           hi - lo, _stream()), "wr_narrow_ids_i64")
                     cols = h["ids32"]
                 plan = self.ops.GroupPlan(cols[0][lo:hi], cols[1][lo:hi], cols[2][lo:hi], B, h["n_users"], h["n_items"],
-                                          arena=h["garenas"][h["tag"]], defer=True)
+                                          arena=h["garenas"][h["tag"]], defer=True, after=first > 0)
                 h["tag"] ^= 1
                 h["next"] = (first, plan)
                 return
@@ -1659,6 +1687,10 @@
         words = tabs.sticky_words()
         if not words:
             return
+        self._check_sticky(h)
+        h["sticky_pending"] = self._copy_sticky(h, words, main)
+
+    def _copy_sticky(self, h, words, main):
         pin = h.get("sticky_pin")
         if pin is None or pin.numel() < 2 * len(words):
             pin = h["sticky_pin"] = torch.zeros(2 * max(len(words), 4), dtype=torch.int32, pin_memory=True)
@@ -1669,8 +1701,7 @@
             pin[off + j:off + j + 1].copy_(wd, non_blocking=True)
         ev = torch.cuda.Event()
         ev.record(main)
-        self._check_sticky(h)
-        h["sticky_pending"] = (ev, pin[off:off + len(words)])
+        return (ev, pin[off:off + len(words)])
 
     def _check_sticky(self, h):
         pend = h.pop("sticky_pending", None)
@@ -1680,7 +1711,6 @@
                 raise abi.WhisprRecHipError(self.STICKY_MSG)
 
     def _take_next(self, h, pos, main):
-        self._check_sticky(h)
         if h["next"] is None:
             self._prefetch(h)
         cur = h["next"]
@@ -1689,6 +1719,9 @@
         plan.validate()
         if isinstance(plan, GroupPlan):
             if plan.overflow or plan.long_run:
+                if "open" in h:
+                    self._close_chain(h, main)
+                    self._queue_sticky(h, h["open_tabs"], main)
                 h["group"] = False
                 self.stats["group_fallbacks"] += 1
                 if h["next"] is not None and h["next"][0] != cur[0]:
@@ -1726,8 +1759,55 @@
         h["cur"], h["next"] = cur, None
         return cur
 
+    def _close_chain(self, h, main):
+        carry = h.pop("open", None)
+        if carry is None:
+            return
+        plan = carry.keep[0]
+        h["open_tabs"].run_sgd_group_stream(plan, 0, 0, h["open_lr"], losses=carry.keep[1], carry=carry, close=True)
+        if carry.batch == plan.n_batches - 1:
+            plan.arena.release_after(main)
+
+    def _run_group_steps(self, h, tabs, plan, first, c, lr, losses, close, main):
+        carry = h.pop("open", None)
+        before = carry.keep[0] if carry is not None else None
+        release = None
+        if before is not None and before is not plan:
+            pool = h.setdefault("release_events", [])
+            if len(pool) < 4:
+                pool.append(torch.cuda.Event(enable_timing=True))
+                pool[-1].record(self.plan_stream)
+            release = pool[h.get("release_at", 0) % len(pool)]
+            h["release_at"] = h.get("release_at", 0) + 1
+        h["open_tabs"], h["open_lr"] = tabs, lr
+        try:
+            _, h["open"] = tabs.run_sgd_group_stream(plan, first, c, lr, losses=losses, carry=carry, close=close,
+                                                     carried_read=release)
+        except BaseException:
+            h["open"] = carry
+            raise
+        if release is not None:
+            before.arena.free = release
+            words = tabs.sticky_words()
+            if words:
+                self._check_sticky(h)
+                with torch.cuda.stream(self.plan_stream):
+                    self.plan_stream.wait_event(release)
+                    h["sticky_pending"] = self._copy_sticky(h, words, self.plan_stream)
+                self._check_sticky(h)
+        if close and first + c == plan.n_batches:
+            plan.arena.release_after(main)
+        if h["open"] is None:
+            h.pop("open")
+
     def _run_span(self, h, sg, pos, end, lr, losses, loss_off):
         main = torch.cuda.current_stream(sg["tabs"].U.device)
+        try:
+            self._run_span_open(h, sg, pos, end, lr, losses, loss_off, main)
+        finally:
+            self._close_chain(h, main)
+
+    def _run_span_open(self, h, sg, pos, end, lr, losses, loss_off, main):
         while pos < end:
             cur = h["cur"]
             if cur is None or pos >= cur[0] + cur[1].n_batches:
@@ -1743,7 +1823,11 @@
             elif self.PREFETCH_AFTER_TRIPLETS > 0 and h["next"] is None and h["at"] < h["nb"] and \
                     c > (self.PREFETCH_AFTER_TRIPLETS + h["B"] - 1) // h["B"]:
                 c = (self.PREFETCH_AFTER_TRIPLETS + h["B"] - 1) // h["B"]
-            if isinstance(plan, GroupPlan):
+            grouped = isinstance(plan, GroupPlan)
+            if grouped and h["group"]:
+                self._run_group_steps(h, sg["tabs"], plan, pos - base, c, lr, losses[loss_off:loss_off + c], pos + c >= end, main)
+                self.stats["group_calls"] += 1
+            elif grouped:
                 sg["tabs"].run_sgd_group(plan, pos - base, c, lr, losses=losses[loss_off:loss_off + c])
                 self.stats["group_calls"] += 1
             elif h["runner"] is not None:
@@ -1758,8 +1842,10 @@
             pos += c
             loss_off += c
             if pos >= base + plan.n_batches:
-                plan.arena.release_after(main)
-                self._queue_sticky(h, sg["tabs"], main)
+                if not (grouped and h["group"]):
+                    plan.arena.release_after(main)
+                if "open" not in h:
+                    self._queue_sticky(h, sg["tabs"], main)
             if h["next"] is None and not h["inline"]:
                 self._prefetch(h)
         h["pos"] = pos
```

After: 2.629 billion triplets/s, median of 6. Within noise of the previous version (+1.7%).
